# Parskatt/RoMa

Measured on AMD Instinct MI355X. Metric: image-pairs/sec, roma_outdoor 560->864, batch=8 per GPU, higher is better.
Workload: dtype bf16; 1 GPU; roma_outdoor match() 560->864, symmetric, upsample_preds, 8 pairs/GPU/step, seeded synthetic weights + N(0,1) images; precision policy of the reference's bf16 timing script: bfloat16 DINOv2 + float16 autocast for VGG / decoder / refiners (ROMA_MIXED), f32 accumulate; precision_policy=mixed, global_batch=8, streams_per_gpu=2, parallelism=single GPU, outputs_finite=True

## Files before the change

roma_amd/_lib.py:

```python
from __future__ import annotations

import ctypes as C
import os
import re

import torch

_PKG = os.path.dirname(os.path.abspath(__file__))
_HERE = os.environ.get("ROMA_LIB_DIR", _PKG)
LIB_PATH = os.path.join(_HERE, "libroma_hip.so")
LIB_PATHS = {"bf16": LIB_PATH, "f16": os.path.join(_HERE, "libroma_hip_f16.so")}

ROMA_F32, ROMA_BF16, ROMA_F16, ROMA_MIXED = 0, 1, 2, 3
H16_CODE = {"bf16": ROMA_BF16, "f16": ROMA_F16}


class RomaConfig(C.Structure):
    _fields_ = [("coarse_h", C.c_int), ("coarse_w", C.c_int), ("upsample_h", C.c_int), ("upsample_w", C.c_int),
                ("symmetric", C.c_int), ("upsample_preds", C.c_int), ("attenuate_cert", C.c_int),
                ("precision", C.c_int), ("max_batch", C.c_int), ("device", C.c_int)]


class RomaForwardArgs(C.Structure):
    _fields_ = [("upsample", C.c_int), ("symmetric", C.c_int), ("scale_factor", C.c_double),
                ("seed_flow", C.c_void_p), ("seed_cert", C.c_void_p), ("seed_h", C.c_int), ("seed_w", C.c_int),
                ("flow", C.c_void_p * 5), ("cert", C.c_void_p * 5), ("feat", C.c_void_p * 5)]


_CTYPES = {"int": C.c_int, "long": C.c_long, "float": C.c_float, "double": C.c_double, "long long": C.c_longlong,
           "unsigned long long": C.c_ulonglong, "roma_handle_t": C.c_void_p}


def _ctype(text, named, decl):
    words = re.findall(r"\w+|\*", text) if re.fullmatch(r"[\w\s*]+", text) else []
    if "*" in words:
        return C.c_char_p if [w for w in words[:words.index("*")] if w != "const"] == ["char"] else C.c_void_p
    key = " ".join(w for w in (words[:-1] if named else words) if w != "const")
    if key not in _CTYPES:
        raise ImportError(f"roma_hip.h: no ctypes type for `{' '.join(text.split())}` in `{decl}`")
    return _CTYPES[key]


def parse_header(text):
    text = re.sub(r"/\*.*?\*/|//[^\n]*", " ", text, flags=re.S)
    text = re.sub(r"^[ \t]*#.*$", " ", text, flags=re.M)
    text = re.sub(r"\b(typedef\s+struct|enum)\s*\{[^}]*\}[^;]*;|\btypedef\b[^;{]*;", " ", text)
    text = re.sub(r'extern\s+"C"\s*\{|\}', " ", text)
    sigs = {}
    for decl in filter(None, (" ".join(d.split()) for d in text.split(";"))):
        m = re.fullmatch(r"([\w\s*]+?)\s*\b(\w+)\s*\((.*)\)", decl)
        if not m:
            raise ImportError(f"roma_hip.h: `{decl}` is not a function declaration")
        ret, name, params = m.groups()
        sigs[name] = (_ctype(ret, False, decl), [_ctype(p, True, decl) for p in params.split(",") if params.strip() != "void"])
    return sigs


HEADER_PATH = os.path.join(os.path.dirname(_PKG), "include", "roma_hip.h")
if not os.path.exists(HEADER_PATH):
    raise ImportError(f"{HEADER_PATH} not found - roma_amd reads the signatures of the C ABI from it")
with open(HEADER_PATH) as _f:
    SIGNATURES = parse_header(_f.read())
EXTENSION_HEADERS = [os.path.join(os.path.dirname(_PKG), "include", "roma_hip_registration.h")]
EXTENSIONS = {}
for _path in EXTENSION_HEADERS:
    if not os.path.exists(_path):
        raise ImportError(f"{_path} not found - roma_amd reads the signatures of the C ABI from it")
    with open(_path) as _f:
        _sigs = parse_header(_f.read())
    _twice = sorted(set(_sigs) & (set(SIGNATURES) | set(EXTENSIONS)))
    if _twice:
        raise ImportError(f"{_path} declares {_twice} a second time")
    EXTENSIONS.update(_sigs)

_libs = {}


class RomaHipError(RuntimeError):
    pass


def load(fmt: str = "bf16"):
    if fmt in _libs:
        return _libs[fmt]
    path = LIB_PATHS[fmt]
    if not os.path.exists(path):
        raise ImportError(f"{path} not found - build it with `python -c 'import __graft_entry__ as g; g.build()'` "
                          "(roma_amd has no CPU fallback)")
    lib = C.CDLL(path)
    for name, (res, args) in {**SIGNATURES, **EXTENSIONS}.items():
        fn = getattr(lib, name)
        fn.restype = res
        fn.argtypes = args
    if lib.roma_h16_format() != H16_CODE[fmt]:
        raise ImportError(f"{path} does not store {fmt} (roma_h16_format() = {lib.roma_h16_format()})")
    lib.h16 = fmt
    _libs[fmt] = lib
    return lib


def fmt_of(dtype) -> str:
    return "f16" if str(dtype) == "torch.float16" else "bf16"


def last_error(lib=None) -> str:
    return (lib or load()).roma_last_error().decode("utf-8", "replace")


def check(rc: int, exc=RomaHipError, lib=None):
    if rc != 0:
        raise exc(last_error(lib))
    return rc


def _ptr(t):
    return C.c_void_p(t.data_ptr() if t is not None else 0)


def _stream(dev):
    return C.c_void_p(torch.cuda.current_stream(dev).cuda_stream)


def _device_tensor(x, name, module):
    if not isinstance(x, torch.Tensor) or not x.is_cuda:
        raise RomaHipError(f"roma_amd.{module}: {name} must be a tensor on a HIP device; there is no CPU fallback")
    return x.detach()
```

roma_amd/csrc/conv64.h:

```cpp
#pragma once
#include "gemm.h"

namespace roma {
int conv64_try_launch(const GemmArgs& a, hipStream_t stream);
int conv3x3_c3_bf16_launch(const float* img, const void* w, const float* bias, void* out, int B, int H, int W, hipStream_t stream);
}
```

roma_amd/csrc/conv64.hip:

```cpp
#include "conv64.h"

#include <stdio.h>
#include <stdlib.h>

#include <algorithm>

#include "gemm_device.h"
#include "tuning.h"

namespace roma {

static __device__ __attribute__((aligned(256))) unsigned int g_c64_dump[256];

#define C64_WAIT_VM(N) asm volatile("s_waitcnt vmcnt(%0)" ::"n"(N) : "memory")

template <int COUT>
__global__ __launch_bounds__(256, 2) void conv3x3_c64_kernel(const bf16_t* __restrict__ in, const bf16_t* __restrict__ w,
                                                             const float* __restrict__ bias, bf16_t* __restrict__ out, int B,
                                                             int H, int W, int SY, int nxt, int nblocks) {
  constexpr int NCG = COUT / 32;
  constexpr int NPG = 4 / NCG;
  constexpr int TW = 64 * NPG;
  constexpr int NPIECE = ((TW + 2) * 128 + 1023) / 1024;
  constexpr int RSTRIDE = NPIECE * 1024;
  constexpr int KW = (NPIECE + 3) / 4;
  extern __shared__ __attribute__((aligned(1024))) unsigned char ring[];

  if ((int)blockIdx.x >= nblocks) return;
  const int tid = threadIdx.x, lane = tid & 63;
  const int wave = __builtin_amdgcn_readfirstlane(tid >> 6);
  const int cg = wave % NCG, pg = wave / NCG;
  const int l31 = lane & 31, h = lane >> 5;
  typedef unsigned u32x4 __attribute__((ext_vector_type(4)));
  const unsigned ring0 = (unsigned)(size_t)((__attribute__((address_space(3))) unsigned char*)ring);

  u32x4 wreg[36];
  {
    const bf16_t* wp = w + (long)(32 * cg + l31) * 576 + 8 * h;
#pragma unroll
    for (int ks = 0; ks < 36; ++ks) wreg[ks] = *reinterpret_cast<const u32x4*>(wp + 16 * ks);
  }
  float* bias_s = reinterpret_cast<float*>(ring + 4 * RSTRIDE);
  if (tid < COUT) bias_s[tid] = bias[tid];

  unsigned rdo[3];
#pragma unroll
  for (int dx = 0; dx < 3; ++dx) {
    const int p = 64 * pg + l31 + dx;
    rdo[dx] = ring0 + (unsigned)(p * 128 + ((h ^ ((p >> 1) & 7)) << 4));
  }

  for (int lb = blockIdx.x; lb < nblocks; lb += gridDim.x) {
  const int xt = lb % nxt;
  const int r = lb / nxt;
  const int yt = (H + SY - 1) / SY;
  const int ys = (r % yt) * SY;
  const int b = r / yt;
  const int x0 = xt * TW;
  const int sy = min(SY, H - ys);
  if (lb != (int)blockIdx.x) __builtin_amdgcn_s_barrier();

  const bf16_t* inb = in + (long)b * H * W * 64;
  const __amdgpu_buffer_rsrc_t rs_in = __builtin_amdgcn_make_buffer_rsrc(const_cast<bf16_t*>(inb), 0, (int)((long)H * W * 128), 0x00020000);
  unsigned voff[KW];
  bool okx[KW];
  {
    const int dl_p = lane >> 3, dl_slot = lane & 7;
    const u32x4 z4 = {0u, 0u, 0u, 0u};
#pragma unroll
    for (int j = 0; j < KW; ++j) {
      const int q = wave + 4 * j;
      const int p = q * 8 + dl_p;
      const int x = x0 - 1 + p;
      const int c = dl_slot ^ ((p >> 1) & 7);
      okx[j] = q < NPIECE && p < TW + 2 && x >= 0 && x < W;
      voff[j] = okx[j] ? (unsigned)(x * 128 + c * 16) : 0u;
      if (q < NPIECE && !okx[j]) {
        int ln = lane;
        asm volatile("" : "+v"(ln));
#pragma unroll
        for (int sl = 0; sl < 4; ++sl)
          asm volatile("ds_write_b128 %0, %1" ::"v"(ring0 + sl * RSTRIDE + q * 1024 + ln * 16), "v"(z4) : "memory");
      }
    }
  }
  asm volatile("s_waitcnt vmcnt(0) lgkmcnt(0)" ::: "memory");

#define C64_ISSUE_ROW(YY, SLOT)                                                                                \
  {                                                                                                            \
    const int yy_ = (YY);                                                                                      \
    if (yy_ >= 0 && yy_ < H) {                                                                                 \
      const int so_ = yy_ * W * 128;                                                                           \
      _Pragma("unroll") for (int j = 0; j < KW; ++j) {                                                         \
        const int q_ = wave + 4 * j;                                                                           \
        if (q_ < NPIECE) {                                                                                     \
          if (okx[j])                                                                                          \
            __builtin_amdgcn_raw_ptr_buffer_load_lds(rs_in, (__attribute__((address_space(3))) void*)(ring + (SLOT) * RSTRIDE + q_ * 1024), \
                                                     16, (int)voff[j], so_, 0, 0);                             \
        }                                                                                                      \
      }                                                                                                        \
    } else {                                     \
      const u32x4 z4_ = {0u, 0u, 0u, 0u};                                                                      \
      int ln_ = lane;                                                                                          \
      asm volatile("" : "+v"(ln_));                                                                            \
      _Pragma("unroll") for (int j = 0; j < KW; ++j) {                                                         \
        const int q_ = wave + 4 * j;                                                                           \
        if (q_ < NPIECE)                                                                                       \
          asm volatile("ds_write_b128 %0, %1" ::"v"(ring0 + (SLOT) * RSTRIDE + q_ * 1024 + ln_ * 16), "v"(z4_) : "memory"); \
      }                                                                                                        \
    }                                                                                                          \
  }

  u32x4 fa[2][4];
#define C64_READ_G(SLOTOFF, DX, G)                                                                            \
  {                                                                                                           \
    const unsigned ad_ = (rdo[DX] + (SLOTOFF)) ^ (unsigned)((G) << 5);                                         \
    asm volatile("ds_read_b128 %0, %1" : "=v"(fa[0][G]) : "v"(ad_));                                           \
    asm volatile("ds_read_b128 %0, %1 offset:4096" : "=v"(fa[1][G]) : "v"(ad_));                              \
  }
#define C64_WAIT_G(G, N) asm volatile("s_waitcnt lgkmcnt(%2)" : "+v"(fa[0][G]), "+v"(fa[1][G]) : "n"(N) : "memory")

  C64_ISSUE_ROW(ys - 1, 0)
  C64_ISSUE_ROW(ys, 1)
  C64_ISSUE_ROW(ys + 1, 2)

  bf16_t* outb = out + (long)b * H * W * COUT;
  for (int o = 0; o < sy; ++o) {
    if (o == 0) {
      asm volatile("s_waitcnt vmcnt(0) lgkmcnt(0)" ::: "memory");
    } else {
      C64_WAIT_VM(0);
    }
    __builtin_amdgcn_s_barrier();
    C64_ISSUE_ROW(ys + o + 2, (o + 3) & 3)
    if (o == 0) {
      C64_READ_G(0, 0, 0)
      C64_READ_G(0, 0, 1)
    }
    C64_READ_G((o & 3) * RSTRIDE, 0, 2)
    C64_READ_G((o & 3) * RSTRIDE, 0, 3)

    f32x16 acc[2];
#pragma unroll
    for (int tm = 0; tm < 2; ++tm)
#pragma unroll
      for (int e = 0; e < 16; ++e) acc[tm][e] = 0.f;
#pragma unroll
    for (int t = 0; t < 9; ++t) {
#pragma unroll
      for (int g = 0; g < 4; ++g) {
        if (t == 8 && g == 3) {
          C64_WAIT_G(g, 4);
        } else {
          C64_WAIT_G(g, 6);
        }
#pragma unroll
        for (int tm = 0; tm < 2; ++tm)
          acc[tm] = mfma_h16_32x32x16(wreg[t * 4 + g],
                                                            fa[tm][g], acc[tm]);
        __builtin_amdgcn_sched_barrier(0);
        if (t + 1 < 9) {
          C64_READ_G(((o + (t + 1) / 3) & 3) * RSTRIDE, (t + 1) % 3, g)
        } else if (g < 2) {
          C64_READ_G(((o + 1) & 3) * RSTRIDE, 0, g)
        }
        __builtin_amdgcn_sched_barrier(0);
      }
    }

    const int y = ys + o;
#pragma unroll
    for (int P = 0; P < 2; ++P) {
      f32x4 bv0, bv1;
      {
        const unsigned ba = ring0 + 4 * RSTRIDE + (32 * cg + 16 * P + 4 * h) * 4;
        asm volatile("ds_read_b128 %0, %2\n\tds_read_b128 %1, %2 offset:32\n\ts_waitcnt lgkmcnt(0)"
                     : "=&v"(bv0), "=&v"(bv1)
                     : "v"(ba)
                     : "memory");
      }
#pragma unroll
      for (int tm = 0; tm < 2; ++tm) {
        const int x = x0 + 64 * pg + 32 * tm + l31;
        const unsigned a0 = pack_bf16x2(fmaxf(acc[tm][8 * P + 0] + bv0[0], 0.f), fmaxf(acc[tm][8 * P + 1] + bv0[1], 0.f));
        const unsigned a1 = pack_bf16x2(fmaxf(acc[tm][8 * P + 2] + bv0[2], 0.f), fmaxf(acc[tm][8 * P + 3] + bv0[3], 0.f));
        const unsigned b0 = pack_bf16x2(fmaxf(acc[tm][8 * P + 4] + bv1[0], 0.f), fmaxf(acc[tm][8 * P + 5] + bv1[1], 0.f));
        const unsigned b1 = pack_bf16x2(fmaxf(acc[tm][8 * P + 6] + bv1[2], 0.f), fmaxf(acc[tm][8 * P + 7] + bv1[3], 0.f));
        const auto s0 = __builtin_amdgcn_permlane32_swap(a0, b0, false, false);
        const auto s1 = __builtin_amdgcn_permlane32_swap(a1, b1, false, false);
        const u32x4 st = {s0[0], s1[0], s0[1], s1[1]};
        bf16_t* op = outb + ((long)y * W + x) * COUT + 32 * cg + 16 * P + 8 * h;
        u32x4* dst = x < W ? reinterpret_cast<u32x4*>(op) : reinterpret_cast<u32x4*>(g_c64_dump) + lane;
        *dst = st;
      }
    }
  }
  C64_WAIT_VM(0);
  }
#undef C64_WAIT_G
#undef C64_READ_G
#undef C64_ISSUE_ROW
}

template <int DUMMY>
__global__ __launch_bounds__(512, 1) void conv3x3_c128_kernel(const bf16_t* __restrict__ in, const bf16_t* __restrict__ w,
                                                              const float* __restrict__ bias, bf16_t* __restrict__ out, int B,
                                                              int H, int W, int SY, int nxt, int nblocks) {
  constexpr int COUT = 128, TW = 64;
  constexpr int NPIECE = ((TW + 2) * 256 + 1023) / 1024;
  constexpr int RSTRIDE = NPIECE * 1024;
  constexpr int KW = (NPIECE + 7) / 8;
  constexpr int XCH = 4 * RSTRIDE;
  constexpr int BIAS = XCH + 2 * 8 * 4096;
  extern __shared__ __attribute__((aligned(1024))) unsigned char ring[];
  if ((int)blockIdx.x >= nblocks) return;

  const int tid = threadIdx.x, lane = tid & 63;
  const int wave = __builtin_amdgcn_readfirstlane(tid >> 6);
  const int cg = wave & 3, kh = wave >> 2;
  const int l31 = lane & 31, h = lane >> 5;
  typedef unsigned u32x4 __attribute__((ext_vector_type(4)));
  const unsigned ring0 = (unsigned)(size_t)((__attribute__((address_space(3))) unsigned char*)ring);

  u32x4 wreg[36];
  {
    const bf16_t* wp = w + (long)(32 * cg + l31) * 1152 + 64 * kh + 8 * h;
#pragma unroll
    for (int t = 0; t < 9; ++t)
#pragma unroll
      for (int g = 0; g < 4; ++g) wreg[t * 4 + g] = *reinterpret_cast<const u32x4*>(wp + 128 * t + 16 * g);
  }
  float* bias_s = reinterpret_cast<float*>(ring + BIAS);
  if (tid < COUT) bias_s[tid] = bias[tid];

  unsigned rdo[3];
#pragma unroll
  for (int dx = 0; dx < 3; ++dx) {
    const int p = l31 + dx;
    rdo[dx] = ring0 + (unsigned)(p * 256 + (((8 * kh + h) ^ (p & 15)) << 4));
  }
  const unsigned xw = ring0 + XCH + (unsigned)((cg + 4 * (1 - kh)) * 4096 + lane * 16);
  const unsigned xr = ring0 + XCH + (unsigned)((cg + 4 * kh) * 4096 + lane * 16);

  for (int lb = blockIdx.x; lb < nblocks; lb += gridDim.x) {
  const int xt = lb % nxt;
  const int r = lb / nxt;
  const int yt = (H + SY - 1) / SY;
  const int ys = (r % yt) * SY;
  const int b = r / yt;
  const int x0 = xt * TW;
  const int sy = min(SY, H - ys);
  if (lb != (int)blockIdx.x) __builtin_amdgcn_s_barrier();

  const bf16_t* inb = in + (long)b * H * W * 128;
  const __amdgpu_buffer_rsrc_t rs_in = __builtin_amdgcn_make_buffer_rsrc(const_cast<bf16_t*>(inb), 0, (int)((long)H * W * 256), 0x00020000);
  unsigned voff[KW];
  bool okx[KW];
  {
    const int dl_p = lane >> 4, dl_slot = lane & 15;
    const u32x4 z4 = {0u, 0u, 0u, 0u};
#pragma unroll
    for (int j = 0; j < KW; ++j) {
      const int q = wave + 8 * j;
      const int p = q * 4 + dl_p;
      const int x = x0 - 1 + p;
      const int c = dl_slot ^ (p & 15);
      okx[j] = q < NPIECE && p < TW + 2 && x >= 0 && x < W;
      voff[j] = okx[j] ? (unsigned)(x * 256 + c * 16) : 0u;
      if (q < NPIECE && !okx[j]) {
        int ln = lane;
        asm volatile("" : "+v"(ln));
#pragma unroll
        for (int sl = 0; sl < 4; ++sl)
          asm volatile("ds_write_b128 %0, %1" ::"v"(ring0 + sl * RSTRIDE + q * 1024 + ln * 16), "v"(z4) : "memory");
      }
    }
  }
  asm volatile("s_waitcnt vmcnt(0) lgkmcnt(0)" ::: "memory");

#define C128_ISSUE_ROW(YY, SLOT)                                                                               \
  {                                                                                                            \
    const int yy_ = (YY);                                                                                      \
    if (yy_ >= 0 && yy_ < H) {                                                                                 \
      const int so_ = yy_ * W * 256;                                                                           \
      _Pragma("unroll") for (int j = 0; j < KW; ++j) {                                                         \
        const int q_ = wave + 8 * j;                                                                           \
        if (q_ < NPIECE) {                                                                                     \
          if (okx[j])                                                                                          \
            __builtin_amdgcn_raw_ptr_buffer_load_lds(rs_in, (__attribute__((address_space(3))) void*)(ring + (SLOT) * RSTRIDE + q_ * 1024), \
                                                     16, (int)voff[j], so_, 0, 0);                             \
        }                                                                                                      \
      }                                                                                                        \
    } else {                                                                                                   \
      const u32x4 z4_ = {0u, 0u, 0u, 0u};                                                                      \
      int ln_ = lane;                                                                                          \
      asm volatile("" : "+v"(ln_));                                                                            \
      _Pragma("unroll") for (int j = 0; j < KW; ++j) {                                                         \
        const int q_ = wave + 8 * j;                                                                           \
        if (q_ < NPIECE)                                                                                       \
          asm volatile("ds_write_b128 %0, %1" ::"v"(ring0 + (SLOT) * RSTRIDE + q_ * 1024 + ln_ * 16), "v"(z4_) : "memory"); \
      }                                                                                                        \
    }                                                                                                          \
  }

  u32x4 fa[2][4];
#define C128_READ_G(SLOTOFF, DX, G)                                                                           \
  {                                                                                                           \
    const unsigned ad_ = (rdo[DX] + (SLOTOFF)) ^ (unsigned)((G) << 5);                                         \
    asm volatile("ds_read_b128 %0, %1" : "=v"(fa[0][G]) : "v"(ad_));                                           \
    asm volatile("ds_read_b128 %0, %1 offset:8192" : "=v"(fa[1][G]) : "v"(ad_));                              \
  }
#define C128_WAIT_G(G, N) asm volatile("s_waitcnt lgkmcnt(%2)" : "+v"(fa[0][G]), "+v"(fa[1][G]) : "n"(N) : "memory")

  bf16_t* outb = out + (long)b * H * W * COUT;
#define C128_EPILOGUE(ACC, Y, PAR)                                                                            \
  {                                                                                                           \
    f32x4 pp_[4];                                                                                             \
    asm volatile("ds_read_b128 %0, %4\n\tds_read_b128 %1, %4 offset:1024\n\tds_read_b128 %2, %4 offset:2048\n\t" \
                 "ds_read_b128 %3, %4 offset:3072\n\ts_waitcnt lgkmcnt(0)"                                    \
                 : "=&v"(pp_[0]), "=&v"(pp_[1]), "=&v"(pp_[2]), "=&v"(pp_[3])                                 \
                 : "v"(xr + (unsigned)(PAR) * 32768u)                                                         \
                 : "memory");                                                                                 \
    const int x_ = x0 + 32 * kh + l31;                                                                        \
    _Pragma("unroll") for (int P = 0; P < 2; ++P) {                                                           \
      f32x4 bv0_, bv1_;                                                                                       \
      asm volatile("ds_read_b128 %0, %2\n\tds_read_b128 %1, %2 offset:32\n\ts_waitcnt lgkmcnt(0)"            \
                   : "=&v"(bv0_), "=&v"(bv1_)                                                                 \
                   : "v"(ring0 + BIAS + (32 * cg + 16 * P + 4 * h) * 4)                                       \
                   : "memory");                                                                               \
      const f32x4 p0_ = pp_[2 * P], p1_ = pp_[2 * P + 1];                                                     \
      const unsigned a0_ = pack_bf16x2(fmaxf(ACC[8 * P + 0] + p0_[0] + bv0_[0], 0.f), fmaxf(ACC[8 * P + 1] + p0_[1] + bv0_[1], 0.f)); \
      const unsigned a1_ = pack_bf16x2(fmaxf(ACC[8 * P + 2] + p0_[2] + bv0_[2], 0.f), fmaxf(ACC[8 * P + 3] + p0_[3] + bv0_[3], 0.f)); \
      const unsigned b0_ = pack_bf16x2(fmaxf(ACC[8 * P + 4] + p1_[0] + bv1_[0], 0.f), fmaxf(ACC[8 * P + 5] + p1_[1] + bv1_[1], 0.f)); \
      const unsigned b1_ = pack_bf16x2(fmaxf(ACC[8 * P + 6] + p1_[2] + bv1_[2], 0.f), fmaxf(ACC[8 * P + 7] + p1_[3] + bv1_[3], 0.f)); \
      const auto s0_ = __builtin_amdgcn_permlane32_swap(a0_, b0_, false, false);                              \
      const auto s1_ = __builtin_amdgcn_permlane32_swap(a1_, b1_, false, false);                              \
      const u32x4 st_ = {s0_[0], s1_[0], s0_[1], s1_[1]};                                                     \
      bf16_t* op_ = outb + ((long)(Y) * W + x_) * COUT + 32 * cg + 16 * P + 8 * h;                            \
      u32x4* dst_ = x_ < W ? reinterpret_cast<u32x4*>(op_) : reinterpret_cast<u32x4*>(g_c64_dump) + lane;     \
      *dst_ = st_;                                                                                            \
    }                                                                                                         \
  }
#define C128_PUBLISH(ACC, PAR)                                                                                \
  _Pragma("unroll") for (int j = 0; j < 4; ++j) {                                                             \
    const f32x4 v_ = {ACC[4 * j + 0], ACC[4 * j + 1], ACC[4 * j + 2], ACC[4 * j + 3]};                        \
    asm volatile("ds_write_b128 %0, %1" ::"v"(xw + (unsigned)(PAR) * 32768u + j * 1024), "v"(v_) : "memory"); \
  }

  C128_ISSUE_ROW(ys - 1, 0)
  C128_ISSUE_ROW(ys, 1)
  C128_ISSUE_ROW(ys + 1, 2)

  f32x16 acc[2];
  for (int o = 0; o < sy; ++o) {
    asm volatile("s_waitcnt vmcnt(0) lgkmcnt(0)" ::: "memory");
    __builtin_amdgcn_s_barrier();
    if (o > 0) {
      if (kh == 0) C128_EPILOGUE(acc[0], ys + o - 1, (o - 1) & 1)
      else C128_EPILOGUE(acc[1], ys + o - 1, (o - 1) & 1)
    }
    C128_ISSUE_ROW(ys + o + 2, (o + 3) & 3)
    if (o == 0) {
      C128_READ_G(0, 0, 0)
      C128_READ_G(0, 0, 1)
    }
    C128_READ_G((o & 3) * RSTRIDE, 0, 2)
    C128_READ_G((o & 3) * RSTRIDE, 0, 3)

#pragma unroll
    for (int tm = 0; tm < 2; ++tm)
#pragma unroll
      for (int e = 0; e < 16; ++e) acc[tm][e] = 0.f;
#pragma unroll
    for (int t = 0; t < 9; ++t) {
#pragma unroll
      for (int g = 0; g < 4; ++g) {
        if (t == 8 && g == 3) {
          C128_WAIT_G(g, 4);
        } else {
          C128_WAIT_G(g, 6);
        }
#pragma unroll
        for (int tm = 0; tm < 2; ++tm)
          acc[tm] = mfma_h16_32x32x16(wreg[t * 4 + g],
                                                            fa[tm][g], acc[tm]);
        __builtin_amdgcn_sched_barrier(0);
        if (t + 1 < 9) {
          C128_READ_G(((o + (t + 1) / 3) & 3) * RSTRIDE, (t + 1) % 3, g)
        } else if (g < 2) {
          C128_READ_G(((o + 1) & 3) * RSTRIDE, 0, g)
        }
        __builtin_amdgcn_sched_barrier(0);
      }
    }
    if (kh == 0) C128_PUBLISH(acc[1], o & 1)
    else C128_PUBLISH(acc[0], o & 1)
  }
  asm volatile("s_waitcnt vmcnt(0) lgkmcnt(0)" ::: "memory");
  __builtin_amdgcn_s_barrier();
  if (kh == 0) C128_EPILOGUE(acc[0], ys + sy - 1, (sy - 1) & 1)
  else C128_EPILOGUE(acc[1], ys + sy - 1, (sy - 1) & 1)
  C64_WAIT_VM(0);
  }
#undef C128_PUBLISH
#undef C128_EPILOGUE
#undef C128_WAIT_G
#undef C128_READ_G
#undef C128_ISSUE_ROW
}

__global__ __launch_bounds__(256, 4) void conv3x3_c3_bf16_kernel(const float* __restrict__ img, const bf16_t* __restrict__ w,
                                                                 const float* __restrict__ bias, bf16_t* __restrict__ out, int B,
                                                                 int H, int W, int RY, int nxt, long ntiles) {
  __shared__ __attribute__((aligned(16))) float bias_s[64];
  __shared__ __attribute__((aligned(1024))) unsigned char stage[4][4096];
  if (threadIdx.x < 64) bias_s[threadIdx.x] = bias[threadIdx.x];
  __syncthreads();
  const int lane = threadIdx.x & 63;
  const int wave = __builtin_amdgcn_readfirstlane(threadIdx.x >> 6);
  const long t = (long)blockIdx.x * 4 + wave;
  if (t >= ntiles) return;
  const int xt = (int)(t % nxt);
  const long r = t / nxt;
  const int nyb = (H + RY - 1) / RY;
  const int y0 = (int)(r % nyb) * RY;
  const int b = (int)(r / nyb);
  const int l31 = lane & 31, h = lane >> 5;
  const int x = xt * 32 + l31;
  const int HW = H * W;
  typedef unsigned u32x4 __attribute__((ext_vector_type(4)));

  u32x4 wf[2][2];
#pragma unroll
  for (int cb = 0; cb < 2; ++cb)
#pragma unroll
    for (int ks = 0; ks < 2; ++ks) wf[cb][ks] = *reinterpret_cast<const u32x4*>(w + (32 * cb + l31) * 32 + 16 * h + 8 * ks);

  int toff[16], tsel[16];
#pragma unroll
  for (int s_ = 0; s_ < 16; ++s_) {
    const int k0 = s_, k1 = 16 + s_;
    const int o0 = (k0 / 9) * HW + ((k0 % 9) / 3 - 1) * W + (k0 % 3 - 1);
    const int o1 = k1 < 27 ? (k1 / 9) * HW + ((k1 % 9) / 3 - 1) * W + (k1 % 3 - 1) : 0;
    const int m0 = (1 << ((k0 % 9) / 3)) | (8 << (k0 % 3));
    const int m1 = k1 < 27 ? ((1 << ((k1 % 9) / 3)) | (8 << (k1 % 3))) : 64;
    toff[s_] = h ? o1 : o0;
    tsel[s_] = h ? m1 : m0;
  }
  const int colbits = ((x >= 1 && x - 1 < W) ? 8 : 0) | (x < W ? 16 : 0) | (x + 1 < W ? 32 : 0);
  const bool cols_in = xt * 32 >= 1 && xt * 32 + 33 <= W;
  const float* p0 = img + (long)b * 3 * HW;
  bf16_t* outb = out + (long)b * HW * 64;
  const unsigned st0 = (unsigned)(size_t)((__attribute__((address_space(3))) unsigned char*)stage[wave]);
  const int ny = min(RY, H - y0);
  for (int o = 0; o < ny; ++o) {
    const int y = y0 + o;
    const int base = y * W + x;
    float v[16];
    if (cols_in && y >= 1 && y + 1 < H) {
#pragma unroll
      for (int s_ = 0; s_ < 16; ++s_) v[s_] = p0[base + toff[s_]];
      if (h) {
#pragma unroll
        for (int s_ = 11; s_ < 16; ++s_) v[s_] = 0.f;
      }
    } else {
      const int okbits = colbits | (y >= 1 ? 1 : 0) | 2 | (y + 1 < H ? 4 : 0);
#pragma unroll
      for (int s_ = 0; s_ < 16; ++s_) {
        const bool ok = (okbits & tsel[s_]) == tsel[s_];
        const float ld = p0[ok ? base + toff[s_] : 0];
        v[s_] = ok ? ld : 0.f;
      }
    }
    u32x4 fr[2];
#pragma unroll
    for (int ks = 0; ks < 2; ++ks)
#pragma unroll
      for (int j = 0; j < 4; ++j) fr[ks][j] = pack_bf16x2(v[8 * ks + 2 * j], v[8 * ks + 2 * j + 1]);
    f32x16 acc[2];
#pragma unroll
    for (int cb = 0; cb < 2; ++cb) {
#pragma unroll
      for (int e = 0; e < 16; ++e) acc[cb][e] = 0.f;
#pragma unroll
      for (int ks = 0; ks < 2; ++ks)
        acc[cb] = mfma_h16_32x32x16(wf[cb][ks],
                                                          fr[ks], acc[cb]);
    }
#pragma unroll
    for (int cb = 0; cb < 2; ++cb)
#pragma unroll
      for (int P = 0; P < 2; ++P) {
        const f32x4 b0 = *reinterpret_cast<const f32x4*>(bias_s + 32 * cb + 16 * P + 4 * h);
        const f32x4 b1 = *reinterpret_cast<const f32x4*>(bias_s + 32 * cb + 16 * P + 8 + 4 * h);
        const unsigned a0 = pack_bf16x2(fmaxf(acc[cb][8 * P + 0] + b0[0], 0.f), fmaxf(acc[cb][8 * P + 1] + b0[1], 0.f));
        const unsigned a1 = pack_bf16x2(fmaxf(acc[cb][8 * P + 2] + b0[2], 0.f), fmaxf(acc[cb][8 * P + 3] + b0[3], 0.f));
        const unsigned c0 = pack_bf16x2(fmaxf(acc[cb][8 * P + 4] + b1[0], 0.f), fmaxf(acc[cb][8 * P + 5] + b1[1], 0.f));
        const unsigned c1 = pack_bf16x2(fmaxf(acc[cb][8 * P + 6] + b1[2], 0.f), fmaxf(acc[cb][8 * P + 7] + b1[3], 0.f));
        const auto s0 = __builtin_amdgcn_permlane32_swap(a0, c0, false, false);
        const auto s1 = __builtin_amdgcn_permlane32_swap(a1, c1, false, false);
        const u32x4 st = {s0[0], s1[0], s0[1], s1[1]};
        const int c = 4 * cb + 2 * P + h;
        *reinterpret_cast<__attribute__((address_space(3))) u32x4*>(st0 + l31 * 128 + ((c ^ (l31 & 7)) << 4)) = st;
      }
#pragma unroll
    for (int i = 0; i < 4; ++i) {
      const u32x4 st = *reinterpret_cast<__attribute__((address_space(3))) const u32x4*>(st0 + i * 1024 + lane * 16);
      const int px = i * 8 + (lane >> 3);
      const int c = (lane & 7) ^ (px & 7);
      if (xt * 32 + px < W) *reinterpret_cast<u32x4*>(outb + ((long)y * W + xt * 32 + px) * 64 + c * 8) = st;
    }
  }
}

int conv3x3_c3_bf16_launch(const float* img, const void* w, const float* bias, void* out, int B, int H, int W, hipStream_t stream) {
  ROMA_REQUIRE(img && w && bias && out && B > 0 && H > 0 && W > 0, "conv3x3_c3_bf16: bad arguments");
  ROMA_REQUIRE((long)3 * H * W < (1l << 23), "conv3x3_c3_bf16: image too large for the packed tap offsets");
  const int RY = 8;
  const int nxt = (W + 31) / 32;
  const long ntiles = (long)B * ((H + RY - 1) / RY) * nxt;
  ProfScope ps("conv3x3_c3_bf16_kernel", (double)B * H * W * (12.0 + 128.0), "byte", stream);
  hipLaunchKernelGGL(conv3x3_c3_bf16_kernel, dim3((unsigned)((ntiles + 3) / 4)), dim3(256), 0, stream, img,
                     reinterpret_cast<const bf16_t*>(w), bias, reinterpret_cast<bf16_t*>(out), B, H, W, RY, nxt, ntiles);
  ROMA_LAUNCH_CHECK();
  return 0;
}

int conv64_try_launch(const GemmArgs& a, hipStream_t stream) {
  const int use = tuning(SW_CONV64);
  const bool c128 = a.conv_c == 128;
  if (!(use & (c128 ? 2 : 1))) return 1;
  if ((a.conv_c != 64 && !c128) || a.in_dt != DT_BF16 || a.out_dt != DT_BF16 || a.act != ACT_RELU || !a.bias) return 1;
  if (c128 ? a.N != 128 : (a.N != 64 && a.N != 128)) return 1;
  if (a.ldc != a.N || a.ldw != 9 * a.conv_c || a.batch != 1 || a.mode != EPI_STD || a.scale || a.res || a.res_bf16 || a.alpha != 1.0f)
    return 1;
  const int H = a.conv_h, W = a.conv_w;
  const long hw = (long)H * W;
  if (hw <= 0 || a.M % hw != 0) return 1;
  if ((long)hw * a.conv_c * 2 >= (1l << 31)) return 1;
  const int B = (int)(a.M / hw);
  const int TW = (!c128 && a.N == 64) ? 128 : 64;
  const int slots = c128 ? 256 : 512;
  const int sy_env = tuning(SW_CONV64_SY);
  const int nxt = (W + TW - 1) / TW;
  int SY = sy_env;
  if (SY <= 0) {
    long best = -1;
    for (int yt = 1; yt <= std::max(1, H / 12); ++yt) {
      const int sy = (H + yt - 1) / yt;
      const long n = (long)B * nxt * ((H + sy - 1) / sy);
      const long cost = ((n + slots - 1) / slots) * (sy + 3);
      if (best < 0 || cost < best) {
        best = cost;
        SY = sy;
      }
    }
  }
  const long nb = (long)B * ((H + SY - 1) / SY) * nxt;
  if (nb <= 0 || nb >= (1l << 30)) return 1;
  char pname[64];
  snprintf(pname, sizeof pname, c128 ? "conv3x3_c128_kernel<%d>" : "conv3x3_c64_kernel<%d>", a.N);
  ProfScope ps(pname, 2.0 * (double)a.M * a.N * 9.0 * a.conv_c, "flop", stream);
  const bf16_t* in = reinterpret_cast<const bf16_t*>(a.A);
  const bf16_t* w = reinterpret_cast<const bf16_t*>(a.W);
  bf16_t* out = reinterpret_cast<bf16_t*>(a.C);
  constexpr int LDS64 = 4 * 17 * 1024 + 512, LDS64N128 = 4 * 9 * 1024 + 512;
  constexpr int LDS128 = 4 * 17 * 1024 + 2 * 8 * 4096 + 512;
  static bool attr_set[64] = {false};
  int dev = 0;
  ROMA_CHECK_HIP(hipGetDevice(&dev));
  if (dev < 0 || dev >= 64 || !attr_set[dev]) {
    ROMA_CHECK_HIP(hipFuncSetAttribute(reinterpret_cast<const void*>(&conv3x3_c64_kernel<64>), hipFuncAttributeMaxDynamicSharedMemorySize, LDS64));
    ROMA_CHECK_HIP(hipFuncSetAttribute(reinterpret_cast<const void*>(&conv3x3_c64_kernel<128>), hipFuncAttributeMaxDynamicSharedMemorySize, LDS64N128));
    ROMA_CHECK_HIP(hipFuncSetAttribute(reinterpret_cast<const void*>(&conv3x3_c128_kernel<0>), hipFuncAttributeMaxDynamicSharedMemorySize, LDS128));
    if (dev >= 0 && dev < 64) attr_set[dev] = true;
  }
  const long gx = std::min<long>(nb, slots);
  if (c128) {
    hipLaunchKernelGGL(conv3x3_c128_kernel<0>, dim3((unsigned)gx), dim3(512), LDS128, stream, in, w, a.bias, out, B, H, W, SY, nxt, (int)nb);
  } else if (a.N == 64) {
    hipLaunchKernelGGL(conv3x3_c64_kernel<64>, dim3((unsigned)gx), dim3(256), LDS64, stream, in, w, a.bias, out, B, H, W, SY, nxt, (int)nb);
  } else {
    hipLaunchKernelGGL(conv3x3_c64_kernel<128>, dim3((unsigned)gx), dim3(256), LDS64N128, stream, in, w, a.bias, out, B, H, W, SY, nxt, (int)nb);
  }
  ROMA_LAUNCH_CHECK();
  return 0;
}

}
```

roma_amd/csrc/model.hip:

```cpp
#include "model.h"

#include <dlfcn.h>
#include <math.h>
#include <stdlib.h>

#include <algorithm>

#include "arch.h"
#include "attention.h"
#include "conv64.h"
#include "dry_run.h"
#include "pool_proj.h"
#include "elementwise.h"
#include "gemm.h"
#include "gp.h"
#include "local_corr.h"
#include "refiner_block.h"
#include "vit.h"

namespace roma {

std::mutex g_peer_mutex;
extern void* g_peer_lib;
extern int g_mixed_handles;

Model::~Model() {
  for (int i = 0; i < MAX_STREAMS - 1; ++i) {
    if (side[i]) (void)hipStreamDestroy(side[i]);
    if (ev_join[i]) (void)hipEventDestroy(ev_join[i]);
  }
  if (ev_fork) (void)hipEventDestroy(ev_fork);
  for (void* p : owned) (void)hipFree(p);
  for (auto& kv : dbg) (void)hipFree(kv.second.first);
  for (auto& kv : inject) (void)hipFree(kv.second.first);
  if (peer_lib) {
    std::lock_guard<std::mutex> lk(g_peer_mutex);
    --g_mixed_handles;
  }
}


int Model::load_peer() {
  static void* lib = nullptr;
  static int (*fwd)(const roma_vit_args_t*, void*) = nullptr;
  std::lock_guard<std::mutex> lk(g_peer_mutex);
  if (!lib) {
    ROMA_REQUIRE(roma_h16_format() == ROMA_F16, "ROMA_MIXED is a mode of the binary16 build (libroma_hip_f16.so)");
    Dl_info info;
    ROMA_REQUIRE(dladdr(reinterpret_cast<void*>(&roma_vit_forward), &info) && info.dli_fname, "ROMA_MIXED: cannot locate this library");
    std::string path(info.dli_fname);
    const size_t slash = path.find_last_of('/');
    path = (slash == std::string::npos ? std::string("") : path.substr(0, slash + 1)) + "libroma_hip.so";
    void* l = dlopen(path.c_str(), RTLD_NOW | RTLD_LOCAL | RTLD_DEEPBIND);
    if (!l) {
      set_error("ROMA_MIXED: cannot load the bfloat16 library " + path + ": " + (dlerror() ? dlerror() : "?"));
      return ROMA_ERR_STATE;
    }
    auto fmt = reinterpret_cast<int (*)(void)>(dlsym(l, "roma_h16_format"));
    auto self = reinterpret_cast<int (*)(void)>(dlsym(l, "roma_self_check"));
    auto abi = reinterpret_cast<int (*)(void)>(dlsym(l, "roma_abi_stamp"));
    auto f = reinterpret_cast<int (*)(const roma_vit_args_t*, void*)>(dlsym(l, "roma_vit_forward"));
    std::string why;
    if (!fmt || !f || !self || !abi) why = "it does not export roma_h16_format / roma_self_check / roma_abi_stamp / roma_vit_forward (an older build)";
    else if (fmt() != ROMA_BF16) why = "it is not the bfloat16 build";
    else if (abi() != roma_abi_stamp()) why = "its ABI stamp " + std::to_string(abi()) + " differs from this library's " + std::to_string(roma_abi_stamp()) + " (stale build: roma_vit_args_t would be misread)";
    else if (self() != ROMA_BF16) why = "its internal calls resolve into another library (symbol interposition: link both builds with -Wl,-Bsymbolic)";
    if (!why.empty()) {
      dlclose(l);
      set_error("ROMA_MIXED: " + path + " cannot serve as the bfloat16 sibling: " + why);
      return ROMA_ERR_STATE;
    }
    lib = l;
    fwd = f;
    g_peer_lib = l;
  }
  if (!peer_lib) ++g_mixed_handles;
  peer_lib = lib;
  peer_vit_forward = fwd;
  return 0;
}

int Model::debug_inject(const char* name, const void* host, size_t bytes) {
  ROMA_REQUIRE(name, "roma_debug_inject: null name");
  const std::string k(name);
  ROMA_REQUIRE(k == "gm_flow16" || k == "gm_cert16", "roma_debug_inject: unknown stage (gm_flow16, gm_cert16)");
  ROMA_CHECK_HIP(hipSetDevice(cfg.device));
  auto it = inject.find(k);
  if (it != inject.end()) {
    ROMA_CHECK_HIP(hipDeviceSynchronize());
    (void)hipFree(it->second.first);
    inject.erase(it);
  }
  if (!host || bytes == 0) return 0;
  void* p = nullptr;
  ROMA_CHECK_HIP(hipMalloc(&p, bytes));
  ROMA_CHECK_HIP(hipMemcpy(p, host, bytes, hipMemcpyHostToDevice));
  inject[k] = {p, bytes};
  return 0;
}

int Model::finalize() {
  ROMA_REQUIRE(!finalized, "roma_finalize: already finalized");
  ROMA_CHECK_HIP(hipSetDevice(cfg.device));
  if (int rc = check_contract()) return rc;
  act_dt = cfg.precision == ROMA_F32 ? DT_F32 : DT_BF16;
  mixed = cfg.precision == ROMA_MIXED;
  if (mixed)
    if (int rc = load_peer()) return rc;
  if (int rc = pack_weights()) return rc;
  host.clear();
  arena.dry = persist.dry = true;
  arena.peak = persist.peak = 0;
  const int keep_sym = cfg.symmetric, keep_up = cfg.upsample_preds;
  cfg.symmetric = 1;
  cfg.upsample_preds = cfg.upsample_h > 0 ? 1 : 0;
  int rc = match_impl(cfg.max_batch, nullptr, nullptr, nullptr, nullptr, nullptr, nullptr, nullptr, true, arena, persist);
  int cf[5];
  for (int i = 0; i < 5; ++i) cf[i] = ref[i].Cf;
  pack = pack_layout(cfg.coarse_h, cfg.coarse_w, cfg.upsample_h, cfg.upsample_w, cf, act_dt == DT_F32 ? 4 : 2);
  const EncodedIn plan_enc;
  if (!rc) rc = match_impl(cfg.max_batch, nullptr, nullptr, nullptr, nullptr, nullptr, nullptr, nullptr, true, arena, persist, nullptr, &plan_enc);
  if (!rc) rc = encode_impl(2 * cfg.max_batch, nullptr, nullptr, nullptr, nullptr, true, cfg.upsample_h > 0, arena, persist);
  Arena plan, plan_p;
  if (!rc && cfg.max_batch >= 2)
    rc = match_impl(cfg.max_batch / 2, nullptr, nullptr, nullptr, nullptr, nullptr, nullptr, nullptr, true, plan, plan_p);
  if (!rc && cfg.max_batch >= 2)
    rc = match_impl(cfg.max_batch / 2, nullptr, nullptr, nullptr, nullptr, nullptr, nullptr, nullptr, true, plan, plan_p, nullptr, &plan_enc);
  cfg.symmetric = keep_sym;
  cfg.upsample_preds = keep_up;
  if (rc) return rc;
  side_arena_bytes = plan.peak + 4096;
  side_persist_bytes = plan_p.peak + 4096;
  arena.cap = arena.peak + 4096;
  persist.cap = persist.peak + 4096;
  ROMA_CHECK_HIP(hipMalloc((void**)&arena.base, arena.cap));
  owned.push_back(arena.base);
  ROMA_CHECK_HIP(hipMalloc((void**)&persist.base, persist.cap));
  owned.push_back(persist.base);
  ROMA_CHECK_HIP(hipMemset(persist.base, 0, persist.cap));
  ROMA_CHECK_HIP(hipMemset(arena.base, 0, arena.cap));
  arena.dry = persist.dry = false;
  finalized = true;
  return 0;
}

int Model::ensure_side_streams(int n) {
  for (int i = streams_ready - 1; i + 1 < n; ++i) {
    Arena &a = side_arena[i], &p = side_persist[i];
    a.cap = side_arena_bytes;
    p.cap = side_persist_bytes;
    ROMA_CHECK_HIP(hipMalloc((void**)&a.base, a.cap));
    owned.push_back(a.base);
    ROMA_CHECK_HIP(hipMalloc((void**)&p.base, p.cap));
    owned.push_back(p.base);
    ROMA_CHECK_HIP(hipMemset(p.base, 0, p.cap));
    ROMA_CHECK_HIP(hipMemset(a.base, 0, a.cap));
    ROMA_CHECK_HIP(hipDeviceSynchronize());
    a.dry = p.dry = false;
    ROMA_CHECK_HIP(hipStreamCreateWithFlags(&side[i], hipStreamNonBlocking));
    ROMA_CHECK_HIP(hipEventCreateWithFlags(&ev_join[i], hipEventDisableTiming));
    if (!ev_fork) ROMA_CHECK_HIP(hipEventCreateWithFlags(&ev_fork, hipEventDisableTiming));
    streams_ready = i + 2;
  }
  return 0;
}

static int dbg_dual_slot() { return tuning(SW_DEBUG_DUAL_SLOT); }

int Model::dbg_save(const char* name, const void* p, size_t bytes, hipStream_t st) {
  if (!debug) return 0;
  if (dbg_dual_slot() >= 0) {
    static const std::string only = std::string(",") + (getenv("ROMA_DEBUG_ONLY") ? getenv("ROMA_DEBUG_ONLY") : "") + ",";
    if (dbg_cur_slot != dbg_dual_slot() || only.find(std::string(",") + name + ",") == std::string::npos) return 0;
  }
  auto it = dbg.find(name);
  if (it == dbg.end() || it->second.second != bytes) {
    if (it != dbg.end()) (void)hipFree(it->second.first);
    void* q = nullptr;
    ROMA_CHECK_HIP(hipMalloc(&q, bytes));
    dbg[name] = {q, bytes};
    it = dbg.find(name);
  }
  ROMA_CHECK_HIP(hipMemcpyAsync(it->second.first, p, bytes, hipMemcpyDeviceToDevice, st));
  return 0;
}

int Model::match(int B, const float* ima, const float* imb, const float* ima_hr, const float* imb_hr, float* warp,
                 float* cert, hipStream_t st) {
  ROMA_REQUIRE(finalized, "roma_match: call roma_finalize first");
  ROMA_REQUIRE(B >= 1 && B <= cfg.max_batch, "roma_match: batch size out of range (max_batch)");
  ROMA_REQUIRE(ima && imb && warp && cert, "roma_match: null image / output pointer");
  if (cfg.upsample_preds) {
    ROMA_REQUIRE(cfg.upsample_h > 0, "roma_match: upsample_preds set but the handle has no upsample resolution");
    ROMA_REQUIRE(ima_hr && imb_hr, "roma_match: upsample_preds requires im_A_high_res and im_B_high_res");
  }
  ROMA_CHECK_HIP(hipSetDevice(cfg.device));
  return match_streams(B, ima, imb, ima_hr, imb_hr, warp, cert, st);
}

int Model::forward(int B, const float* ima, const float* imb, const roma_forward_args_t* fw, hipStream_t st) {
  ROMA_REQUIRE(finalized, "roma_forward: call roma_finalize first");
  ROMA_REQUIRE(B >= 1 && B <= cfg.max_batch, "roma_forward: batch size out of range (max_batch)");
  ROMA_REQUIRE(ima && imb && fw, "roma_forward: null image / argument pointer");
  if (fw->upsample) {
    ROMA_REQUIRE(cfg.upsample_h > 0, "roma_forward: upsample pass on a handle without an upsample resolution");
    ROMA_REQUIRE(fw->seed_flow && fw->seed_cert && fw->seed_h > 0 && fw->seed_w > 0,
                 "roma_forward: the upsample pass needs batch[\"corresps\"] (seed_flow / seed_cert)");
  }
  ROMA_CHECK_HIP(hipSetDevice(cfg.device));
  return match_impl(B, ima, imb, nullptr, nullptr, nullptr, nullptr, st, false, arena, persist, fw);
}

int Model::encode(int N, const float* images, const float* images_hr, void* feats, long feats_bytes, hipStream_t st) {
  ROMA_REQUIRE(finalized, "roma_encode: call roma_finalize first");
  ROMA_REQUIRE(N >= 1 && images && feats, "roma_encode: N < 1 or null image / feature pointer");
  ROMA_REQUIRE(!images_hr || cfg.upsample_h > 0, "roma_encode: high-resolution images on a handle without an upsample resolution");
  ROMA_REQUIRE(feats_bytes == (long)N * pack.total, "roma_encode: feats_bytes must be N * roma_encoded_bytes() = " +
                                                        std::to_string((long)N * pack.total) + " (got " + std::to_string(feats_bytes) + ")");
  ROMA_REQUIRE((reinterpret_cast<uintptr_t>(feats) & 15) == 0, "roma_encode: the feature buffer must be 16-byte aligned");
  ROMA_CHECK_HIP(hipSetDevice(cfg.device));
  const size_t im_lo = (size_t)3 * cfg.coarse_h * cfg.coarse_w, im_hi = (size_t)3 * cfg.upsample_h * cfg.upsample_w;
  const int chunk = 2 * cfg.max_batch;
  for (int i0 = 0; i0 < N; i0 += chunk)
    if (int rc = encode_impl(std::min(chunk, N - i0), images + i0 * im_lo, images_hr ? images_hr + i0 * im_hi : nullptr,
                             static_cast<char*>(feats) + (long)i0 * pack.total, st, false, images_hr != nullptr, arena, persist))
      return rc;
  return 0;
}

int Model::match_encoded(int P, const void* feats, long feats_bytes, int N, const int* idx_a, const int* idx_b, float* warp, float* cert,
                         hipStream_t st) {
  ROMA_REQUIRE(finalized, "roma_match_encoded: call roma_finalize first");
  ROMA_REQUIRE(P >= 1 && P <= cfg.max_batch, "roma_match_encoded: number of pairs out of range (max_batch)");
  ROMA_REQUIRE(feats && idx_a && idx_b && warp && cert && N >= 1, "roma_match_encoded: null pointer or N < 1");
  ROMA_REQUIRE(feats_bytes == (long)N * pack.total, "roma_match_encoded: feats_bytes must be N * roma_encoded_bytes() = " +
                                                        std::to_string((long)N * pack.total) + " (got " + std::to_string(feats_bytes) + ")");
  ROMA_REQUIRE((reinterpret_cast<uintptr_t>(feats) & 15) == 0, "roma_match_encoded: the feature buffer must be 16-byte aligned");
  for (int i = 0; i < P; ++i)
    ROMA_REQUIRE(idx_a[i] >= 0 && idx_a[i] < N && idx_b[i] >= 0 && idx_b[i] < N,
                 "roma_match_encoded: pair " + std::to_string(i) + " = (" + std::to_string(idx_a[i]) + ", " + std::to_string(idx_b[i]) +
                     ") names an image outside [0, " + std::to_string(N) + ")");
  if (cfg.upsample_preds)
    ROMA_REQUIRE(cfg.upsample_h > 0, "roma_match_encoded: upsample_preds set but the handle has no upsample resolution");
  ROMA_CHECK_HIP(hipSetDevice(cfg.device));
  const EncodedIn enc{static_cast<const char*>(feats), idx_a, idx_b};
  return match_streams(P, nullptr, nullptr, nullptr, nullptr, warp, cert, st, &enc);
}

int Model::match_streams(int B, const float* ima, const float* imb, const float* ima_hr, const float* imb_hr, float* warp,
                         float* cert, hipStream_t st, const EncodedIn* enc) {
  const int env_streams = tuning(SW_STREAMS);
  const bool serial_env = tuning(SW_STREAMS_SERIAL) != 0;
  const int ns = (debug && dbg_dual_slot() < 0) ? 1 : std::min(std::min(env_streams > 0 ? env_streams : n_streams, (int)MAX_STREAMS), B);
  if (ns <= 1) return match_impl(B, ima, imb, ima_hr, imb_hr, warp, cert, st, false, arena, persist, nullptr, enc);
  if (int rc = ensure_side_streams(ns)) return rc;
  const size_t im_lo = (size_t)3 * cfg.coarse_h * cfg.coarse_w, im_hi = (size_t)3 * cfg.upsample_h * cfg.upsample_w;
  const int Ho = cfg.upsample_preds ? cfg.upsample_h : cfg.coarse_h, Wo = cfg.upsample_preds ? cfg.upsample_w : cfg.coarse_w;
  const size_t px = (size_t)Ho * Wo * (cfg.symmetric ? 2 : 1);
  ROMA_CHECK_HIP(hipEventRecord(ev_fork, st));
  int rc = 0, b0 = 0;
  for (int i = 0; i < ns; ++i) {
    const int bi = B / ns + (i < B % ns ? 1 : 0);
    hipStream_t si = i == 0 ? st : side[i - 1];
    if (i > 0) ROMA_CHECK_HIP(hipStreamWaitEvent(si, ev_fork, 0));
    if (i > 0 && serial_env) {
      hipStream_t sp = i == 1 ? st : side[i - 2];
      ROMA_CHECK_HIP(hipEventRecord(ev_join[i - 1], sp));
      ROMA_CHECK_HIP(hipStreamWaitEvent(si, ev_join[i - 1], 0));
    }
    EncodedIn sub;
    if (enc) sub = EncodedIn{enc->feats, enc->idx_a + b0, enc->idx_b + b0};
    if (!rc)
      rc = match_impl(bi, ima ? ima + b0 * im_lo : nullptr, imb ? imb + b0 * im_lo : nullptr, ima_hr ? ima_hr + b0 * im_hi : nullptr,
                      imb_hr ? imb_hr + b0 * im_hi : nullptr, warp + b0 * px * 4, cert + b0 * px, si, false,
                      i == 0 ? arena : side_arena[i - 1], i == 0 ? persist : side_persist[i - 1], nullptr, enc ? &sub : nullptr);
    b0 += bi;
  }
  for (int i = 1; i < ns; ++i) {
    (void)hipEventRecord(ev_join[i - 1], side[i - 1]);
    (void)hipStreamWaitEvent(st, ev_join[i - 1], 0);
  }
  return rc;
}

struct Model::Call {
  Arena &arena, &persist;
  int B = 0, nimg = 0, ndp = 0;
  int shift = 0;
  bool sym = false;
  size_t esz = 4;
  hipStream_t st = nullptr;
  bool dry = false;
  int tslot = 0;
  bool tracing = false;
  const roma_forward_args_t* fw = nullptr;
  int th = 0, tw = 0, T = 0;
  int Npd = 0, Npt = 0;
  void *qbuf = nullptr, *kbuf = nullptr, *vtbuf = nullptr;
  void *ln = nullptr, *ao = nullptr, *hid = nullptr;
  Call(Arena& a, Arena& p) : arena(a), persist(p) {}
  void* alloc(size_t elems, size_t es) const { return arena.alloc(elems * es); }
  void* at(void* p, long elems) const { return static_cast<char*>(p) + elems * (long)esz; }
};

struct Model::Pass {
  bool up = false;
  int H = 0, W = 0;
  const float *imA = nullptr, *imB = nullptr;
  void* feat[5] = {nullptr};
  void* pf_pre[2] = {nullptr, nullptr};
  bool pp_on[2] = {false, false};
  double scale_factor = 1.0;
  float *flow = nullptr, *cert = nullptr, *flow_alt = nullptr, *cert_alt = nullptr;
  const char* tag() const { return up ? "p2" : "p1"; }
};

struct Model::Scale {
  int si, ins, hs, ws;
  int lvl;
  long hw, M;
  const RefinerW& r;
  int ldf;
  float sx, sy;
  std::string tp;
  size_t pf_bytes, d_bytes, flow_bytes, cert_bytes;
  void* pf = nullptr;
  void *d0 = nullptr, *d1 = nullptr;
  Scale(const Call& c, const Pass& p, int si_, const RefinerW& r_)
      : si(si_), ins(SCALE_INT[si_]), hs(ins == 16 ? c.th : p.H / ins), ws(ins == 16 ? c.tw : p.W / ins),
        lvl(ins == 16 ? 4 : (ins == 8 ? 3 : (ins == 4 ? 2 : (ins == 2 ? 1 : 0)))), hw((long)hs * ws), M((long)c.ndp * hw), r(r_),
        ldf((int)round_up(r_.Cf, 8)), sx((float)ins / (4.0f * (float)p.W)), sy((float)ins / (4.0f * (float)p.H)),
        tp(std::string(p.tag()) + "_s" + SCALES[si_]), pf_bytes((size_t)c.nimg * hw * ldf * c.esz),
        d_bytes((size_t)M * r_.Cp * c.esz), flow_bytes((size_t)M * 2 * 4), cert_bytes((size_t)M * 4) {}
};

int Model::fits(const Call& c) {
  if (c.dry || !(c.arena.overflow || c.persist.overflow)) return 0;
  c.arena.overflow = c.persist.overflow = false;
  set_error("roma_match / roma_forward: the workspace planned by roma_finalize is too small for this call (an option that "
            "changes the buffer plan was switched after roma_finalize); the results of this call are invalid");
  return -5;
}

int Model::observe(const Call& c, const std::string& trace_name, const std::string& dbg_name, const void* p, size_t bytes,
                   long rows, int ld, int c0, int c1) {
  if (c.tracing && !trace_name.empty() && trace_n[c.tslot] < TRACE_MAX) {
    const int k = trace_n[c.tslot]++;
    if ((int)trace_names[c.tslot].size() <= k) trace_names[c.tslot].push_back(trace_name);
    else trace_names[c.tslot][k] = trace_name;
    unsigned long long* out = trace_dev[c.tslot] + k;
    if (int rc = c1 > c0 ? checksum_cols_launch(p, rows, ld, c0, c1, out, c.st) : checksum_launch(p, bytes, out, c.st)) return rc;
  }
  if (debug && !c.dry && !dbg_name.empty()) return dbg_save(dbg_name.c_str(), p, bytes, c.st);
  return 0;
}

int Model::encode_vgg(const Call& c, Pass& p) {
  const bool dry = c.dry; hipStream_t st = c.st;
  const int H = p.H, W = p.W, nimg = c.nimg, B = c.B;
  const size_t esz = c.esz;
  const int fh[4] = {H, H / 2, H / 4, H / 8}, fw_[4] = {W, W / 2, W / 4, W / 8};
  const int fc[4] = {64, 128, 256, 512};
  size_t fbytes[4];
  for (int l = 0; l < 4; ++l) {
    fbytes[l] = (size_t)nimg * fh[l] * fw_[l] * fc[l] * esz;
    p.feat[l] = c.arena.alloc(fbytes[l]);
  }
  const int pp_si[2] = {4, 3};
  for (int l = 0; l < 2; ++l) {
    const RefinerW& rr = ref[pp_si[l]];
    const int ldf_l = (int)round_up(rr.Cf, 8);
    p.pp_on[l] = tuning(SW_POOL_PROJ) != 0 && fh[l] >= 2 && fw_[l] >= 2 &&
                 pool_proj_supported(fc[l], rr.Cf, ldf_l, act_dt) && proj[pp_si[l]].b != nullptr;
    if (p.pp_on[l] || dry) p.pf_pre[l] = c.alloc((size_t)nimg * fh[l] * fw_[l] * ldf_l, esz);
    if (!p.pp_on[l] && !dry) p.pf_pre[l] = nullptr;
  }
  const size_t enc_mark = c.arena.mark();
  void* t0 = c.alloc((size_t)nimg * H * W * 64, esz);
  void* t1 = c.alloc((size_t)nimg * (H / 2) * (W / 2) * 64, esz);
  void* col1 = c.alloc((size_t)nimg * H * W * 32, esz);
  if (int rc = fits(c)) return rc;
  if (act_dt == DT_BF16 && (tuning(SW_CONV64) & 4) && (long)3 * H * W < (1l << 23)) {
    RUN(conv3x3_c3_bf16_launch(p.imA, vgg[0].w, vgg[0].b, t0, B, H, W, st));
    if (p.imB) RUN(conv3x3_c3_bf16_launch(p.imB, vgg[0].w, vgg[0].b, c.at(t0, (long)B * H * W * 64), B, H, W, st));
  } else {
    RUN(im2col3x3_c3_launch(p.imA, col1, B, H, W, act_dt, st));
    if (p.imB) RUN(im2col3x3_c3_launch(p.imB, c.at(col1, (long)B * H * W * 32), B, H, W, act_dt, st));
    GemmArgs g;
    g.A = col1; g.lda = 32; g.W = vgg[0].w; g.ldw = vgg[0].ldw; g.C = t0; g.ldc = 64;
    g.M = nimg * H * W; g.N = 64; g.K = 32; g.k_alg = 27; g.in_dt = act_dt; g.out_dt = act_dt; g.bias = vgg[0].b; g.act = ACT_RELU;
    RUN(gemm_launch(g, st));
  }
  auto conv = [&](int li, const void* in, void* out, int h, int w) -> int {
    GemmArgs g;
    g.A = in; g.W = vgg[li].w; g.ldw = vgg[li].ldw; g.C = out; g.ldc = vgg_cout[li];
    g.M = nimg * h * w; g.N = vgg_cout[li]; g.K = 9 * vgg_cin[li];
    g.in_dt = act_dt; g.out_dt = act_dt; g.bias = vgg[li].b; g.act = ACT_RELU;
    g.conv_h = h; g.conv_w = w; g.conv_c = vgg_cin[li]; g.conv_korder = vgg_korder[li];
    RUN(gemm_launch(g, st));
    return 0;
  };
  auto pool = [&](int l, const void* in, void* out) -> int {
    if (p.pp_on[l]) {
      const int si_ = pp_si[l];
      RUN(pool_proj_launch(in, out, p.pf_pre[l], proj[si_].w, proj[si_].ldw, proj[si_].b, ref[si_].Cf, (int)round_up(ref[si_].Cf, 8),
                           nimg, fh[l], fw_[l], fc[l], act_dt, st));
    } else {
      RUN(maxpool2x2_launch(in, out, nimg, fh[l], fw_[l], fc[l], act_dt, st));
    }
    return 0;
  };
  if (int rc = conv(1, t0, p.feat[0], H, W)) return rc;
  if (int rc = pool(0, p.feat[0], t1)) return rc;
  if (int rc = conv(2, t1, t0, H / 2, W / 2)) return rc;
  if (int rc = conv(3, t0, p.feat[1], H / 2, W / 2)) return rc;
  if (int rc = pool(1, p.feat[1], t1)) return rc;
  if (int rc = conv(4, t1, t0, H / 4, W / 4)) return rc;
  if (int rc = conv(5, t0, t1, H / 4, W / 4)) return rc;
  if (int rc = conv(6, t1, t0, H / 4, W / 4)) return rc;
  if (int rc = conv(7, t0, p.feat[2], H / 4, W / 4)) return rc;
  RUN(maxpool2x2_launch(p.feat[2], t1, nimg, H / 4, W / 4, 256, act_dt, st));
  if (int rc = conv(8, t1, t0, H / 8, W / 8)) return rc;
  if (int rc = conv(9, t0, t1, H / 8, W / 8)) return rc;
  if (int rc = conv(10, t1, t0, H / 8, W / 8)) return rc;
  if (int rc = conv(11, t0, p.feat[3], H / 8, W / 8)) return rc;
  c.arena.release(enc_mark);
  static const char* const dbg_names[4] = {"feat1", "feat2", "feat4", "feat8"};
  for (int l = 0; l < 4; ++l)
    if (int rc = observe(c, std::string(p.tag()) + "_" + dbg_names[l], p.up ? "" : dbg_names[l], p.feat[l], fbytes[l])) return rc;
  if (c.fw && !dry)
    for (int l = 0; l < 4; ++l)
      if (c.fw->feat[4 - l]) ROMA_CHECK_HIP(hipMemcpyAsync(c.fw->feat[4 - l], p.feat[l], fbytes[l], hipMemcpyDeviceToDevice, st));
  return 0;
}

int Model::encode_dino(Call& c, Pass& p) {
  const bool dry = c.dry; hipStream_t st = c.st;
  const int nimg = c.nimg, T = c.T;
  const size_t esz = c.esz;
  const long rows_d = (long)nimg * (T + 1), rows_t = (long)c.ndp * T;
  const size_t fbytes = (size_t)nimg * T * 1024 * esz;
  p.feat[4] = c.arena.alloc(fbytes);
  const long rmax = std::max(rows_d, rows_t);
  c.ln = c.alloc((size_t)rmax * 1024, esz);
  c.ao = c.alloc((size_t)rmax * 1024, esz);
  c.hid = c.alloc((size_t)rmax * 4096, esz);
  const size_t dmark = c.arena.mark();
  void* col = c.alloc((size_t)nimg * T * patch.ldw, esz);
  float* pt = (float*)c.alloc((size_t)nimg * T * 1024, 4);
  float* x = (float*)c.alloc((size_t)rows_d * 1024, 4);
  const bool res_f32_env = tuning(SW_VIT_RES_F32) != 0;
  void* xs = nullptr;
  if (act_dt == DT_BF16) xs = c.alloc((size_t)rows_d * 1024, 2);
  void* feat_vit = p.feat[4];
  if (mixed) feat_vit = c.alloc((size_t)nimg * T * 1024, 2);
  if (int rc = fits(c)) return rc;
  if (!dry) {
    roma_vit_block_t blk[24];
    for (int i = 0; i < 24; ++i) blk[i] = dino[i].pub();
    roma_vit_args_t va{};
    va.B = c.B; va.H = p.H; va.W = p.W;
    va.act = act_dt == DT_F32 ? ROMA_F32 : (mixed ? ROMA_BF16 : roma_h16_format());
    va.bf16_residual = act_dt == DT_BF16 && vit_bf16_residual && !res_f32_env;
    va.im_a = p.imA; va.im_b = p.imB;
    va.patch_w = patch.w; va.patch_b = patch.b; va.patch_ldw = patch.ldw;
    va.cls_tok = cls_tok; va.pos_emb = pos_emb;
    va.blocks = blk; va.nblocks = 24;
    va.norm_w = dino_nw; va.norm_b = dino_nb;
    va.col = col; va.pt = pt; va.x = x; va.xs = xs; va.ln = c.ln; va.ao = c.ao; va.hid = c.hid;
    va.q = c.qbuf; va.k = c.kbuf; va.vt = c.vtbuf;
    va.feat_out = feat_vit;
    if (mixed) {
      if (int rc = peer_vit_forward(&va, st)) {
        set_error("ROMA_MIXED: roma_vit_forward of the bfloat16 library failed");
        return rc;
      }
      RUN(convert_from_bf16_launch(feat_vit, p.feat[4], (long)nimg * T * 1024, st));
    } else {
      RUN(vit_forward(va, st));
    }
  }
  c.arena.release(dmark);
  if (int rc = observe(c, "feat16", "feat16", p.feat[4], fbytes)) return rc;
  if (c.fw && !dry && c.fw->feat[0]) ROMA_CHECK_HIP(hipMemcpyAsync(c.fw->feat[0], p.feat[4], fbytes, hipMemcpyDeviceToDevice, st));
  return 0;
}

int Model::seed_upsample_pass(const Call& c, const Pass& p, const float* flow_p1, const float* cert_p1) {
  const bool dry = c.dry;
  const roma_forward_args_t* fw = c.fw;
  const int sh = fw ? fw->seed_h : cfg.coarse_h, sw = fw ? fw->seed_w : cfg.coarse_w;
  RUN(resize_bilinear_launch(fw ? fw->seed_flow : flow_p1, p.flow, c.ndp, sh, sw, p.H / 8, p.W / 8, 2, c.st));
  RUN(resize_bilinear_launch(fw ? fw->seed_cert : cert_p1, p.cert, c.ndp, sh, sw, p.H / 8, p.W / 8, 1, c.st));
  return 0;
}

int Model::proj_head(const Call& c, const Pass& p, Scale& s) {
  const bool dry = c.dry;
  const bool pf_ready = s.lvl < 2 && p.pp_on[s.lvl];
  s.pf = pf_ready ? p.pf_pre[s.lvl] : c.arena.alloc(s.pf_bytes);
  if (int rc = fits(c)) return rc;
  if (!pf_ready) {
    GemmArgs g;
    g.A = p.feat[s.lvl]; g.lda = PROJ_CIN[s.si]; g.W = proj[s.si].w; g.ldw = proj[s.si].ldw; g.C = s.pf; g.ldc = s.ldf;
    g.M = (int)(c.nimg * s.hw); g.N = s.r.Cf; g.K = PROJ_CIN[s.si]; g.in_dt = act_dt; g.out_dt = act_dt; g.bias = proj[s.si].b;
    RUN(gemm_launch(g, c.st));
  }
  return observe(c, s.tp + "_proj", s.ins == 16 ? "proj16" : "", s.pf, s.pf_bytes);
}

int Model::coarse_match(const Call& c, const Pass& p, const Scale& s) {
  const bool dry = c.dry; hipStream_t st = c.st;
  const long rows_t = s.M;
  float* tokens = (float*)c.alloc((size_t)rows_t * 1024, 4);
  const size_t gp_mark = c.arena.mark();
  if (int rc = gp_posterior(s.pf, s.ldf, act_dt, c.B, c.sym, c.th, c.tw, gp_w, gp_b, tokens, 1024, c.arena, st, dry))
    return c.arena.overflow ? fits(c) : rc;
  c.arena.release(gp_mark);
  const int ldl = 4104;
  float* logits = (float*)c.alloc((size_t)rows_t * ldl, 4);
  if (int rc = fits(c)) return rc;
  RUN(copy2d_launch(s.pf, s.ldf, act_dt, tokens + 512, 1024, DT_F32, rows_t, 512, st));
  if (int rc = observe(c, "", "tokens16", tokens, (size_t)rows_t * 1024 * 4)) return rc;
  VitScratch sc;
  sc.ln = c.ln; sc.ao = c.ao; sc.hid = c.hid; sc.q = c.qbuf; sc.k = c.kbuf; sc.vt = c.vtbuf;
  for (int i = 0; i < 5; ++i) RUN(vit_block_run(tdec[i].pub(), tokens, DT_F32, rows_t, c.ndp, c.T, c.Npt, 8, 128, 1e-5f, act_dt, sc, st));
  const void* zin = tokens;
  if (act_dt != DT_F32) {
    RUN(copy2d_launch(tokens, 1024, DT_F32, c.ln, 1024, act_dt, rows_t, 1024, st));
    zin = c.ln;
  }
  GemmArgs g;
  g.A = zin; g.lda = 1024; g.W = to_out.w; g.ldw = to_out.ldw; g.C = logits; g.ldc = ldl;
  g.M = (int)rows_t; g.N = to_out.N; g.K = 1024; g.in_dt = act_dt; g.out_dt = DT_F32; g.bias = to_out.b;
  RUN(gemm_launch(g, st));
  if (int rc = observe(c, s.tp + "_tokens_gp", "", tokens, (size_t)rows_t * 1024 * 4)) return rc;
  if (int rc = observe(c, s.tp + "_logits", "logits16", logits, (size_t)rows_t * ldl * 4)) return rc;
  RUN(cls_to_flow_launch(logits, ldl, p.flow, p.cert, rows_t, st));
  if (int rc = observe(c, s.tp + "_gm_flow", "gm_flow16_own", p.flow, s.flow_bytes)) return rc;
  if (!debug || dry) return 0;
  auto inj = [&](const char* nm, float* dst, size_t bytes) -> int {
    auto it = inject.find(nm);
    if (it == inject.end()) return 0;
    ROMA_REQUIRE(it->second.second == bytes, "roma_debug_inject: injected stage has the wrong size for this batch");
    ROMA_CHECK_HIP(hipMemcpyAsync(dst, it->second.first, bytes, hipMemcpyDeviceToDevice, st));
    return 0;
  };
  if (int rc = inj("gm_flow16", p.flow, s.flow_bytes)) return rc;
  if (int rc = inj("gm_cert16", p.cert, s.cert_bytes)) return rc;
  if (int rc = observe(c, "", "gm_flow16", p.flow, s.flow_bytes)) return rc;
  return observe(c, "", "gm_cert16", p.cert, s.cert_bytes);
}

int Model::refiner_input(const Call& c, const Pass& p, Scale& s) {
  const bool dry = c.dry; hipStream_t st = c.st;
  const RefinerW& r = s.r;
  s.d0 = c.arena.alloc(s.d_bytes);
  s.d1 = c.arena.alloc(s.d_bytes);
  LocalCorrArgs lc;
  if (r.radius) {
    const long lc_ints = local_corr_ws_ints(c.ndp, s.hs, s.ws, r.radius);
    lc.ws = (int*)c.alloc((size_t)lc_ints, 4); lc.ws_bytes = lc_ints * 4;
  }
  if (int rc = fits(c)) return rc;
  if (int rc = observe(c, s.tp + "_flow_before", "", p.flow, s.flow_bytes)) return rc;
  RefinerInputArgs ia;
  ia.feat = s.pf; ia.ldf = s.ldf; ia.flow = p.flow; ia.d = s.d0; ia.ldd = r.Cp; ia.emb_w = r.emb_w; ia.emb_b = r.emb_b;
  ia.B = c.ndp; ia.H = s.hs; ia.W = s.ws; ia.C = r.Cf; ia.E = r.E; ia.Kcorr = r.K; ia.nimg = c.nimg; ia.shift = c.shift;
  ia.disp_scale = (float)(40.0 / 32.0 * p.scale_factor); ia.dt = act_dt;
  RUN(refiner_input_launch(ia, st));
  if (r.radius) {
    lc.f0 = s.pf; lc.f1 = s.pf; lc.warp = p.flow; lc.out = c.at(s.d0, 2 * r.Cf + r.E);
    lc.B = c.ndp; lc.H = s.hs; lc.W = s.ws; lc.C = r.Cf; lc.radius = r.radius; lc.ld0 = s.ldf; lc.ld1 = s.ldf; lc.ldo = r.Cp;
    lc.nimg = c.nimg; lc.f1_shift = c.shift; lc.scale = 1.0f / sqrtf((float)r.Cf); lc.in_dt = act_dt; lc.out_dt = act_dt;
    RUN(local_corr_window_launch(lc, st));
  }
  const bool dual = dbg_dual_slot() >= 0;
  const bool din_small = s.d_bytes <= ((size_t)(dual ? 512 : 64) << 20);
  if (int rc = observe(c, s.tp + "_din", din_small ? std::string(p.tag()) + "_din" + SCALES[s.si] : "", s.d0, s.d_bytes)) return rc;
  if (dual && s.ins == 1)
    if (int rc = observe(c, "", std::string(p.tag()) + "_flowin1", p.flow, s.flow_bytes)) return rc;
  if (!c.tracing) return 0;
  if (int rc = observe(c, s.tp + "_proj_again", "", s.pf, s.pf_bytes)) return rc;
  if (int rc = observe(c, s.tp + "_flow_again", "", p.flow, s.flow_bytes)) return rc;
  if (int rc = observe(c, s.tp + "_din_again", "", s.d0, s.d_bytes)) return rc;
  if (c.esz != 2 || r.E <= 0) return 0;
  const int cols[5] = {0, r.Cf, 2 * r.Cf, 2 * r.Cf + r.E, r.Cp};
  static const char* const part[4] = {"_din_x", "_din_xhat", "_din_emb", "_din_rest"};
  for (int i = 0; i < 4; ++i)
    if (int rc = observe(c, s.tp + part[i], "", s.d0, 0, s.M, r.Cp, cols[i], cols[i + 1])) return rc;
  for (int b = 0; b < c.ndp; ++b)
    if (int rc = observe(c, s.tp + "_din_pair" + std::to_string(b), "", c.at(s.d0, (long)b * s.hw * r.Cp), 0, s.hw, r.Cp, 0, r.Cp)) return rc;
  return 0;
}

int Model::refiner_chain(const Call& c, const Pass& p, const Scale& s, const void** d_last, bool* composed) {
  const bool dry = c.dry; hipStream_t st = c.st;
  const RefinerW& r = s.r;
  const bool fused = fuse_refiner_blocks && refiner_block_supported(r.Cp, act_dt);
  float* delta = fused && (dry || compose_out_conv) ? (float*)c.alloc((size_t)s.M * 4, 4) : nullptr;
  if (int rc = fits(c)) return rc;
  void *dcur = s.d0, *dalt = s.d1;
  *composed = compose_out_conv;
  for (int b = 0; b < 9; ++b) {
    const bool last = b == 8 && compose_out_conv;
    if (last && fused) {
      RUN(refiner_block_final_launch(dcur, delta, r.dw_w[b], r.dw_b[b], r.ocf_w, r.Cp, r.ocf_b, c.ndp, s.hs, s.ws, r.Cp, act_dt, st));
      RUN(refiner_apply_delta_launch(delta, p.flow, p.cert, s.M, s.sx, s.sy, st));
      *d_last = nullptr;
      return 0;
    }
    if (fused) {
      RUN(refiner_block_launch(dcur, dalt, r.dw_w[b], r.dw_b[b], r.pw[b].w, r.pw[b].ldw, r.pw[b].b, c.ndp, s.hs, s.ws, r.Cp, act_dt, st));
      std::swap(dcur, dalt);
      if (int rc = observe(c, s.tp + "_blk" + std::to_string(b), "", dcur, s.d_bytes)) return rc;
      continue;
    }
    RUN(dwconv5x5_launch(dcur, dalt, r.dw_w[b], r.dw_b[b], c.ndp, s.hs, s.ws, r.Cp, act_dt, st));
    if (int rc = observe(c, s.tp + "_dw" + std::to_string(b), "", dalt, s.d_bytes)) return rc;
    if (last) {
      std::swap(dcur, dalt);
      break;
    }
    GemmArgs g;
    g.A = dalt; g.lda = r.Cp; g.W = r.pw[b].w; g.ldw = r.pw[b].ldw; g.C = dcur; g.ldc = r.Cp;
    g.M = (int)s.M; g.N = r.Cp; g.K = r.Cp; g.in_dt = act_dt; g.out_dt = act_dt; g.bias = r.pw[b].b;
    g.n_alg = g.k_alg = r.C;
    RUN(gemm_launch(g, st));
    if (int rc = observe(c, s.tp + "_blk" + std::to_string(b), "", dcur, s.d_bytes)) return rc;
  }
  *d_last = dcur;
  return 0;
}

int Model::refiner_out(const Call& c, const Pass& p, const Scale& s, const void* d_last, bool composed) {
  const bool dry = c.dry; hipStream_t st = c.st;
  const RefinerW& r = s.r;
  if (d_last)
    RUN(refiner_out_launch(d_last, r.Cp, act_dt, composed ? r.oc_w : r.out_w, composed ? r.oc_b : r.out_b, p.flow, p.cert, s.M, r.Cp,
                           s.sx, s.sy, st));
  if (int rc = observe(c, s.tp + "_flow", std::string(p.tag()) + "_flow" + SCALES[s.si], p.flow, s.flow_bytes)) return rc;
  if (int rc = observe(c, s.tp + "_cert", std::string(p.tag()) + "_cert" + SCALES[s.si], p.cert, s.cert_bytes)) return rc;
  if (c.fw && !dry) {
    if (c.fw->flow[s.si]) ROMA_CHECK_HIP(hipMemcpyAsync(c.fw->flow[s.si], p.flow, s.flow_bytes, hipMemcpyDeviceToDevice, st));
    if (c.fw->cert[s.si]) ROMA_CHECK_HIP(hipMemcpyAsync(c.fw->cert[s.si], p.cert, s.cert_bytes, hipMemcpyDeviceToDevice, st));
  }
  return 0;
}

int Model::next_scale(const Call& c, Pass& p, const Scale& s, float* cert16_keep) {
  const bool dry = c.dry; hipStream_t st = c.st;
  if (s.ins == 16) {
    if (s.M % 4 == 0) {
      RUN(copy2d_launch(p.cert, s.M, DT_F32, cert16_keep, s.M, DT_F32, 1, (int)s.M, st));
    } else if (!dry) {
      ROMA_CHECK_HIP(hipMemcpyAsync(cert16_keep, p.cert, s.cert_bytes, hipMemcpyDeviceToDevice, st));
    }
  }
  if (s.ins == 1) return 0;
  const int nh = p.H / (s.ins / 2), nw = p.W / (s.ins / 2);
  RUN(resize_bilinear_launch(p.flow, p.flow_alt, c.ndp, s.hs, s.ws, nh, nw, 2, st));
  RUN(resize_bilinear_launch(p.cert, p.cert_alt, c.ndp, s.hs, s.ws, nh, nw, 1, st));
  std::swap(p.flow, p.flow_alt);
  std::swap(p.cert, p.cert_alt);
  return observe(c, s.tp + "_flow_up", "", p.flow, (size_t)c.ndp * nh * nw * 2 * 4);
}

int Model::epilogue(const Call& c, const float* flow, const float* cert, const float* cert16_keep, float* warp_out, float* cert_out) {
  const bool dry = c.dry;
  const int Hfin = cfg.upsample_preds ? cfg.upsample_h : cfg.coarse_h, Wfin = cfg.upsample_preds ? cfg.upsample_w : cfg.coarse_w;
  FinalArgs fa;
  fa.flow = flow;
  fa.cert = cert;
  fa.cert16 = cfg.attenuate_cert ? cert16_keep : nullptr;
  fa.warp = warp_out; fa.certainty = cert_out;
  fa.B = c.B; fa.H = Hfin; fa.W = Wfin; fa.h16 = c.th; fa.w16 = c.tw; fa.symmetric = cfg.symmetric;
  RUN(final_epilogue_launch(fa, c.st));
  const size_t px = (size_t)c.B * Hfin * Wfin * (cfg.symmetric ? 2 : 1);
  if (int rc = observe(c, "final_warp", "", warp_out, px * 4 * 4)) return rc;
  return observe(c, "final_cert", "", cert_out, px * 4);
}

void Model::token_grid(Call& c) {
  c.th = cfg.coarse_h / 14; c.tw = cfg.coarse_w / 14; c.T = c.th * c.tw;
  c.Npd = (int)round_up(c.T + 1, 128); c.Npt = (int)round_up(c.T, 128);
  const size_t qkv_elems = std::max((size_t)c.nimg * 16 * c.Npd * 64, (size_t)c.ndp * 8 * c.Npt * 128);
  c.qbuf = c.persist.alloc(qkv_elems * c.esz);
  c.kbuf = c.persist.alloc(qkv_elems * c.esz);
  c.vtbuf = c.persist.alloc(qkv_elems * c.esz);
}

int Model::decoder_scratch(Call& c) {
  const long rows_t = (long)c.ndp * c.T;
  c.ln = c.alloc((size_t)rows_t * 1024, c.esz);
  c.ao = c.alloc((size_t)rows_t * 1024, c.esz);
  c.hid = c.alloc((size_t)rows_t * 4096, c.esz);
  return fits(c);
}

int Model::gather_head(const Call& c, const Pass& p, Scale& s, const EncodedIn& enc) {
  const bool dry = c.dry;
  s.pf = c.arena.alloc(s.pf_bytes);
  if (int rc = fits(c)) return rc;
  const long seg = pack.off[p.up ? 1 : 0][s.si], slab = pack.bytes[p.up ? 1 : 0][s.si];
  ROMA_REQUIRE(seg >= 0 && (size_t)slab * c.nimg == s.pf_bytes, "roma_match_encoded: the pack layout does not hold this scale");
  for (int i0 = 0; i0 < c.nimg && !dry; i0 += SLAB_MAX) {
    SlabTable t;
    t.n = std::min((int)SLAB_MAX, c.nimg - i0);
    for (int k = 0; k < t.n; ++k) {
      const int i = i0 + k;
      t.src_idx[k] = i < c.B ? enc.idx_a[i] : enc.idx_b[i - c.B];
      t.dst_idx[k] = i;
    }
    RUN(slab_copy_launch(enc.feats + seg, pack.total, s.pf, slab, slab, t, c.st));
  }
  return observe(c, s.tp + "_proj", s.ins == 16 ? "proj16" : "", s.pf, s.pf_bytes);
}

int Model::scatter_head(const Call& c, const Pass& p, const Scale& s, char* feats) {
  const bool dry = c.dry;
  const long seg = pack.off[p.up ? 1 : 0][s.si], slab = pack.bytes[p.up ? 1 : 0][s.si];
  ROMA_REQUIRE(seg >= 0 && (size_t)slab * c.nimg == s.pf_bytes, "roma_encode: the pack layout does not hold this scale");
  for (int i0 = 0; i0 < c.nimg && !dry; i0 += SLAB_MAX) {
    SlabTable t;
    t.n = std::min((int)SLAB_MAX, c.nimg - i0);
    for (int k = 0; k < t.n; ++k) t.src_idx[k] = t.dst_idx[k] = i0 + k;
    RUN(slab_copy_launch(s.pf, slab, feats + seg, pack.total, slab, t, c.st));
  }
  return 0;
}

int Model::encode_impl(int n, const float* im, const float* im_hr, char* feats, hipStream_t st, bool dry, bool with_up, Arena& arena,
                       Arena& persist) {
  Call c(arena, persist);
  c.B = n; c.nimg = n; c.shift = 0; c.sym = false; c.ndp = 0;
  c.esz = act_dt == DT_F32 ? 4 : 2;
  c.st = st; c.dry = dry;
  arena.reset();
  persist.reset();
  dbg_cur_slot = 0;
  token_grid(c);
  if (int rc = fits(c)) return rc;
  for (int pass = 0; pass < (with_up ? 2 : 1); ++pass) {
    Pass p;
    p.up = pass == 1;
    p.H = p.up ? cfg.upsample_h : cfg.coarse_h; p.W = p.up ? cfg.upsample_w : cfg.coarse_w;
    p.imA = p.up ? im_hr : im;
    const size_t pass_mark = arena.mark();
    if (int rc = encode_vgg(c, p)) return rc;
    if (!p.up)
      if (int rc = encode_dino(c, p)) return rc;
    for (int si = p.up ? 1 : 0; si < 5; ++si) {
      Scale s(c, p, si, ref[si]);
      const size_t scale_mark = arena.mark();
      if (int rc = proj_head(c, p, s)) return rc;
      if (int rc = scatter_head(c, p, s, feats)) return rc;
      arena.release(scale_mark);
    }
    arena.release(pass_mark);
  }
  return 0;
}

int Model::match_impl(int B, const float* ima, const float* imb, const float* ima_hr, const float* imb_hr,
                      float* warp_out, float* cert_out, hipStream_t st, bool dry, Arena& arena, Arena& persist,
                      const roma_forward_args_t* fw, const EncodedIn* enc) {
  Call c(arena, persist);
  c.B = B; c.nimg = 2 * B; c.shift = B;
  c.sym = fw ? fw->symmetric != 0 : cfg.symmetric != 0;
  c.ndp = c.sym ? 2 * B : B;
  c.esz = act_dt == DT_F32 ? 4 : 2;
  c.st = st; c.dry = dry; c.fw = fw;
  arena.reset();
  persist.reset();
  c.tslot = (&arena == &this->arena) ? 0 : (int)(&arena - side_arena) + 1;
  dbg_cur_slot = c.tslot;
  c.tracing = trace_on && !dry;
  if (c.tracing) {
    if (!trace_dev[c.tslot]) {
      ROMA_CHECK_HIP(hipMalloc((void**)&trace_dev[c.tslot], TRACE_MAX * sizeof(unsigned long long)));
      owned.push_back(trace_dev[c.tslot]);
    }
    ROMA_CHECK_HIP(hipMemsetAsync(trace_dev[c.tslot], 0, TRACE_MAX * sizeof(unsigned long long), st));
    trace_n[c.tslot] = 0;
  }
  token_grid(c);

  float* cert16_keep = (float*)c.alloc((size_t)c.ndp * c.T, 4);
  float *pp_flow[2][2] = {{nullptr, nullptr}, {nullptr, nullptr}}, *pp_cert[2][2] = {{nullptr, nullptr}, {nullptr, nullptr}};
  for (int ps = 0; ps < ((cfg.upsample_preds || (fw && fw->upsample)) ? 2 : 1); ++ps) {
    const size_t px = (size_t)c.ndp * (ps ? cfg.upsample_h : cfg.coarse_h) * (ps ? cfg.upsample_w : cfg.coarse_w);
    for (int i = 0; i < 2; ++i) {
      pp_flow[ps][i] = (float*)c.alloc(px * 2, 4);
      pp_cert[ps][i] = (float*)c.alloc(px, 4);
    }
  }
  if (int rc = fits(c)) return rc;
  float *flow_p1 = nullptr, *cert_p1 = nullptr;
  float *flow_fin = nullptr, *cert_fin = nullptr;

  const int pass0 = fw ? (fw->upsample ? 1 : 0) : 0, pass1 = fw ? pass0 + 1 : (cfg.upsample_preds ? 2 : 1);
  for (int pass = pass0; pass < pass1; ++pass) {
    Pass p;
    p.up = pass == 1;
    p.H = p.up ? cfg.upsample_h : cfg.coarse_h; p.W = p.up ? cfg.upsample_w : cfg.coarse_w;
    p.imA = (p.up && !fw) ? ima_hr : ima;
    p.imB = (p.up && !fw) ? imb_hr : imb;
    p.scale_factor = sqrt((double)p.H * (double)p.W / (560.0 * 560.0));
    if (!p.up && coarse_scale_factor > 0.0) p.scale_factor = coarse_scale_factor;
    if (fw && fw->scale_factor > 0.0) p.scale_factor = fw->scale_factor;
    p.flow = pp_flow[pass][0]; p.cert = pp_cert[pass][0]; p.flow_alt = pp_flow[pass][1]; p.cert_alt = pp_cert[pass][1];

    const size_t pass_mark = arena.mark();
    if (enc) {
      if (!p.up)
        if (int rc = decoder_scratch(c)) return rc;
    } else {
      if (int rc = encode_vgg(c, p)) return rc;
      if (!p.up)
        if (int rc = encode_dino(c, p)) return rc;
    }
    if (p.up)
      if (int rc = seed_upsample_pass(c, p, flow_p1, cert_p1)) return rc;
    for (int si = p.up ? 1 : 0; si < 5; ++si) {
      Scale s(c, p, si, ref[si]);
      const size_t scale_mark = arena.mark();
      if (int rc = enc ? gather_head(c, p, s, *enc) : proj_head(c, p, s)) return rc;
      if (s.ins == 16) {
        const size_t coarse_mark = arena.mark();
        if (int rc = coarse_match(c, p, s)) return rc;
        arena.release(coarse_mark);
      }
      const void* d_last = nullptr;
      bool composed = false;
      if (int rc = refiner_input(c, p, s)) return rc;
      if (int rc = refiner_chain(c, p, s, &d_last, &composed)) return rc;
      if (int rc = refiner_out(c, p, s, d_last, composed)) return rc;
      arena.release(scale_mark);
      if (int rc = next_scale(c, p, s, cert16_keep)) return rc;
    }
    flow_fin = p.flow; cert_fin = p.cert;
    if (!p.up) { flow_p1 = p.flow; cert_p1 = p.cert; }
    arena.release(pass_mark);
  }
  if (fw) return 0;
  return epilogue(c, flow_fin, cert_fin, cert16_keep, warp_out, cert_out);
}

}
```

roma_amd/csrc/tuning.hip:

```cpp
#include "tuning.h"

#include <stdlib.h>
#include <string.h>

#include "../../include/roma_hip.h"

namespace roma {
void set_error(const std::string& msg);
namespace {

struct Row {
  Switch id;
  const char* key;
  const char* env;
  long def;
  int floor;
  const char* doc;
};

constexpr Row ROWS[] = {
    {SW_GEMM8P, "gemm8p", "ROMA_GEMM8P", 1, 0, "large bf16 GEMMs on the 8-phase 256 x 256 kernel (1) or on the one-barrier-per-slab kernel (0)"},
    {SW_GEMM_DBG, "gemm_dbg", "ROMA_GEMM_DBG", 0, 0, "experiment bits of the GEMM kernels (1 skip output stores, 2 skip the K loop, 2048 no streaming stores, ...)"},
    {SW_GEMM8P_WALK, "gemm8p_walk", nullptr, -1, 1, "gemm8p: tile rows per group of the persistent walk (1 = row major); unset = 8 from 24 tile columns on, else 1"},
    {SW_GEMM8P_SCHED, "gemm8p_sched", "ROMA_GEMM8P_SCHED", 1, 0, "gemm8p K-loop schedule: 1 k-half phases, 0 quadrant phases (tools builds only)"},
    {SW_GEMM8P_MAXWG, "gemm8p_maxwg", nullptr, -1, 8, "gemm8p, measurement only: cap the persistent grid at n workgroups (a multiple of 8); unset = one per CU"},
    {SW_WS1X1, "ws1x1", "ROMA_WS1X1", 1, 0, "N = K = 576 refiner 1x1 on the weight-stationary kernel (1) or on the 256 x 192 tile kernel (0)"},
    {SW_LC_MODE, "lc_mode", "ROMA_LC_MODE", 0, 0, "local correlation: 0 tiled form + gather work list, 1 every tile on the gather list (key only), 2 per-pixel kernel"},
    {SW_LC_BIN, "lc_bin", "ROMA_LC_BIN", 1, 0, "local correlation: queries of incoherent tiles sorted by target bin, counters in LDS (1) or device atomics (2), or gathered per query (0)"},
    {SW_CONV64, "conv64", "ROMA_CONV64", 7, 0, "weight-stationary VGG front end, bit mask: 1 the Cin = 64 kernels, 2 the Cin = 128 kernel, 4 the fused first layer"},
    {SW_CONV_PATCH, "conv_patch", "ROMA_CONV_PATCH", 1, 0, "patch-resident 3x3 kernel for slab-major VGG layers (1) or gemm8p (0); environment 0 also packs tap-major weights"},
    {SW_ATTN_XCD, "attn_xcd", "ROMA_ATTN_XCD", 1, 0, "attention work items in per-XCD bands of (batch, head) (1) or in plain order (0)"},
    {SW_ATTN_EXP2, "attn_exp2", nullptr, -1, 0, "tools only: force the 2^x softmax of the 16-bit attention kernel on / off; unset = as the caller says"},
    {SW_DW_RING, "dw_ring", "ROMA_DW_RING", 1, 0, "depthwise 5x5: 0 register-prefetch kernel, 1 ring kernel for the large launches, 2 ring kernel for every shape it takes"},
    {SW_GP_COL, "gp_col", "ROMA_GP_COL", 1, 0, "GP Cholesky left-looking, one launch per block column (1) or the right-looking launch chain (0)"},
    {SW_POOL_PROJ, "pool_proj", "ROMA_POOL_PROJ", 1, 0, "max-pool + proj head of strides 1 / 2 in one pass (1) or as separate kernels (0)"},
    {SW_GP_COL_LEADER, "gp_col_leader", "ROMA_GP_COL_LEADER", 1, 0, "block-column Cholesky: a leader workgroup factorises the diagonal block, its product formed one launch ahead (1) or in its own launch (2), or every workgroup its own copy (0)"},
    {SW_GEMM8P_MINM, nullptr, "ROMA_GEMM8P_MINM", 2048, 0, "gemm8p: smallest M it takes for the wide (N >= 2048) dense launches"},
    {SW_GEMM_NT, nullptr, "ROMA_GEMM_NT", 1, 0, "non-temporal output stores in the 16-bit GEMM row writer"},
    {SW_GEMM_F32_FILL, nullptr, "ROMA_GEMM_F32_FILL", 1, 0, "exact-f32 GEMMs below 192 tiles of 256 x 256 run on 128 x 128 tiles"},
    {SW_GEMM_SMALLM, nullptr, "ROMA_GEMM_SMALLM", 1, 0, "GEMMs below 320 tiles of 128 x 128 run on 128 x 64 tiles"},
    {SW_CONV64_SY, nullptr, "ROMA_CONV64_SY", 0, 0, "conv64 strip height in rows; 0 = the split of H with the fewest rounds"},
    {SW_CONV_KORDER, nullptr, "ROMA_CONV_KORDER", 1, 0, "VGG layers with Cout >= 256 pack slab-major weight rows (read when a handle is created)"},
    {SW_RB_SY, nullptr, "ROMA_RB_SY", 0, 0, "fused refiner block strip height in rows; 0 = the split of H with the fewest rounds"},
    {SW_DWR_MAXSY, nullptr, "ROMA_DWR_MAXSY", 1 << 20, 0, "depthwise ring kernel: cap of the strip height in rows (at least 6)"},
    {SW_DW_RING_MINELEMS, nullptr, "ROMA_DW_RING_MINELEMS", 64l << 20, 0, "dw_ring = 1: smallest launch, in elements, that goes to the ring kernel"},
    {SW_RI_VEC, nullptr, "ROMA_RI_VEC", 1, 0, "refiner_input on the 16-byte vector kernel where alignment allows"},
    {SW_OUT_ROW, nullptr, "ROMA_OUT_ROW", 1, 0, "refiner_out: row kernel for C = 24 in 16-bit storage"},
    {SW_OUT_LPR, nullptr, "ROMA_OUT_LPR", 1, 0, "refiner_out, 16-bit: lanes per row chosen to fill the 16-byte pieces best"},
    {SW_OUT_ROWS_IT, nullptr, "ROMA_OUT_ROWS_IT", 0, 0, "refiner_out: row groups per wave (even, >= 2); otherwise 8"},
    {SW_GP_AUG, nullptr, "ROMA_GP_AUG", 1, 0, "GP Cholesky: right-hand sides stored behind A ride along the factorisation (0 = separate forward loop)"},
    {SW_GP_BWD2, nullptr, "ROMA_GP_BWD2", 1, 0, "GP Cholesky: backward substitution with one launch per step (0 = two)"},
    {SW_COMPOSE_OUT, nullptr, "ROMA_COMPOSE_OUT", 1, 0, "initial value of the handle option compose_out_conv (read when a handle is created)"},
    {SW_VIT_RES_F32, nullptr, "ROMA_VIT_RES_F32", 0, 0, "force DINOv2's f32 residual stream in the 16-bit modes"},
    {SW_STREAMS, nullptr, "ROMA_STREAMS", 0, 0, "number of sub-batch streams of match(); 0 = the handle's option"},
    {SW_STREAMS_SERIAL, nullptr, "ROMA_STREAMS_SERIAL", 0, 0, "diagnostic: sub-batch streams run one after the other"},
    {SW_DEBUG_DUAL_SLOT, nullptr, "ROMA_DEBUG_DUAL_SLOT", -1, 0, "diagnostic: keep the stream split in debug mode, sub-batch k captures the stages of ROMA_DEBUG_ONLY"},
};
constexpr int NROWS = sizeof(ROWS) / sizeof(ROWS[0]);
constexpr bool rows_in_enum_order() {
  for (int i = 0; i < NROWS; ++i)
    if (ROWS[i].id != i) return false;
  return true;
}
static_assert(NROWS == SW_COUNT && rows_in_enum_order(), "one row per Switch, in enum order");
constexpr bool json_plain(const char* s) {
  for (; s && *s; ++s)
    if (*s == '"' || *s == '\\' || *s < ' ') return false;
  return true;
}
constexpr bool rows_json_plain() {
  for (const Row& r : ROWS)
    if (!json_plain(r.key) || !json_plain(r.env) || !json_plain(r.doc)) return false;
  return true;
}
static_assert(rows_json_plain(), "keys, environment names and docs: plain ASCII without quote, backslash or control character");

struct Overrides {
  long v[SW_COUNT];
  constexpr Overrides() : v{} {
    for (long& x : v) x = -1;
  }
};
[[clang::require_constant_initialization]] Overrides g_override;

struct Env {
  long v[SW_COUNT];
  Env() {
    for (int i = 0; i < NROWS; ++i) {
      const char* s = ROWS[i].env ? getenv(ROWS[i].env) : nullptr;
      v[i] = s ? atol(s) : ROWS[i].def;
    }
  }
};
const Env& env() {
  static const Env e;
  return e;
}

}

long tuning_env(Switch id) { return env().v[id]; }
long tuning_override(Switch id) { return g_override.v[id] >= ROWS[id].floor ? g_override.v[id] : -1; }
long tuning(Switch id) { return g_override.v[id] >= ROWS[id].floor ? g_override.v[id] : tuning_env(id); }

int tuning_set(const char* key, long value) {
  for (const Row& r : ROWS)
    if (r.key && !strcmp(r.key, key)) {
      g_override.v[r.id] = value >= r.floor ? value : -1;
      return 0;
    }
  set_error(std::string("roma_tuning: unknown key ") + key);
  return ROMA_ERR_ARG;
}

std::string tuning_describe() {
  std::string js = "[";
  for (const Row& r : ROWS) {
    const auto quoted = [](const char* s) { return s ? "\"" + std::string(s) + "\"" : std::string("null"); };
    const long ov = tuning_override(r.id);
    js += std::string(r.id ? ", " : "") + "{\"key\": " + quoted(r.key) + ", \"env\": " + quoted(r.env) +
          ", \"default\": " + std::to_string(r.def) + ", \"override\": " + (ov >= 0 ? std::to_string(ov) : "null") +
          ", \"value\": " + std::to_string(tuning(r.id)) + ", \"doc\": " + quoted(r.doc) + "}";
  }
  return js + "]";
}

}
```

Baseline: 109.7 image-pairs/s.

## Fuse VGG conv1_1 into the weight-stationary conv1_2 kernel

Adds a fused VGG front-end kernel that computes the 3-channel conv1_1 on the fly, per row strip, inside the weight-stationary Cin=64 conv1_2 kernel. The row-pipelined conv body moves into a shared template header parameterised on a FRONT mode. This removes the intermediate 64-channel full-resolution activation write and read between the two layers, plus one launch. The cost is extra per-block recomputation of conv1_1 on halo columns and rows. It also adds a C entry point that chains the fused front end with pool_proj.

After: 110.2 image-pairs/s, median of 6. No clear change (+0.5%).

```diff
diff --git a/include/roma_hip_vgg_front.h b/include/roma_hip_vgg_front.h
--- /dev/null
+++ b/include/roma_hip_vgg_front.h
@@ -0,0 +1,14 @@
+#ifndef ROMA_HIP_VGG_FRONT_H
+#define ROMA_HIP_VGG_FRONT_H
+#ifdef __cplusplus
+extern "C" {
+#endif
+
+int roma_op_vgg_front(const float* im_a, const float* im_b, const void* w1, const float* b1, const void* w2, const float* b2,
+                      const void* pw, long ldw, const float* pb, int N, int ldf, void* feat, void* pooled, void* pf, int B, int H,
+                      int W, void* stream);
+
+#ifdef __cplusplus
+}
+#endif
+#endif
diff --git a/roma_amd/_lib.py b/roma_amd/_lib.py
--- a/roma_amd/_lib.py
+++ b/roma_amd/_lib.py
@@ -72,6 +72,13 @@
     if _twice:
         raise ImportError(f"{_path} declares {_twice} a second time")
     EXTENSIONS.update(_sigs)
+VGG_FRONT_HEADER = os.path.join(os.path.dirname(_PKG), "include", "roma_hip_vgg_front.h")
+if not os.path.exists(VGG_FRONT_HEADER):
+    raise ImportError(f"{VGG_FRONT_HEADER} not found - roma_amd reads the signatures of the C ABI from it")
+with open(VGG_FRONT_HEADER) as _f:
+    VGG_FRONT = parse_header(_f.read())
+if set(VGG_FRONT) & (set(SIGNATURES) | set(EXTENSIONS)):
+    raise ImportError(f"{VGG_FRONT_HEADER} declares {sorted(set(VGG_FRONT) & (set(SIGNATURES) | set(EXTENSIONS)))} a second time")
 
 _libs = {}
 
@@ -88,7 +95,7 @@
         raise ImportError(f"{path} not found - build it with `python -c 'import __graft_entry__ as g; g.build()'` "
                           "(roma_amd has no CPU fallback)")
     lib = C.CDLL(path)
-    for name, (res, args) in {**SIGNATURES, **EXTENSIONS}.items():
+    for name, (res, args) in {**SIGNATURES, **EXTENSIONS, **VGG_FRONT}.items():
         fn = getattr(lib, name)
         fn.restype = res
         fn.argtypes = args
diff --git a/roma_amd/csrc/conv64.h b/roma_amd/csrc/conv64.h
--- a/roma_amd/csrc/conv64.h
+++ b/roma_amd/csrc/conv64.h
@@ -3,5 +3,9 @@
 
 namespace roma {
 int conv64_try_launch(const GemmArgs& a, hipStream_t stream);
+int conv64_strip_rows(int B, int H, int nxt, int slots);
 int conv3x3_c3_bf16_launch(const float* img, const void* w, const float* bias, void* out, int B, int H, int W, hipStream_t stream);
+bool vgg_front_supported(int H, int W);
+int vgg_front_launch(const float* imA, const float* imB, const void* w1, const float* b1, const void* w2, const float* b2, void* out,
+                     int B, int H, int W, hipStream_t stream);
 }
diff --git a/roma_amd/csrc/conv64.hip b/roma_amd/csrc/conv64.hip
--- a/roma_amd/csrc/conv64.hip
+++ b/roma_amd/csrc/conv64.hip
@@ -5,201 +5,17 @@
 
 #include <algorithm>
 
+#include "conv64_rows.h"
 #include "gemm_device.h"
 #include "tuning.h"
 
 namespace roma {
-
-static __device__ __attribute__((aligned(256))) unsigned int g_c64_dump[256];
-
-#define C64_WAIT_VM(N) asm volatile("s_waitcnt vmcnt(%0)" ::"n"(N) : "memory")
 
 template <int COUT>
 __global__ __launch_bounds__(256, 2) void conv3x3_c64_kernel(const bf16_t* __restrict__ in, const bf16_t* __restrict__ w,
                                                              const float* __restrict__ bias, bf16_t* __restrict__ out, int B,
                                                              int H, int W, int SY, int nxt, int nblocks) {
-  constexpr int NCG = COUT / 32;
-  constexpr int NPG = 4 / NCG;
-  constexpr int TW = 64 * NPG;
-  constexpr int NPIECE = ((TW + 2) * 128 + 1023) / 1024;
-  constexpr int RSTRIDE = NPIECE * 1024;
-  constexpr int KW = (NPIECE + 3) / 4;
-  extern __shared__ __attribute__((aligned(1024))) unsigned char ring[];
-
-  if ((int)blockIdx.x >= nblocks) return;
-  const int tid = threadIdx.x, lane = tid & 63;
-  const int wave = __builtin_amdgcn_readfirstlane(tid >> 6);
-  const int cg = wave % NCG, pg = wave / NCG;
-  const int l31 = lane & 31, h = lane >> 5;
-  typedef unsigned u32x4 __attribute__((ext_vector_type(4)));
-  const unsigned ring0 = (unsigned)(size_t)((__attribute__((address_space(3))) unsigned char*)ring);
-
-  u32x4 wreg[36];
-  {
-    const bf16_t* wp = w + (long)(32 * cg + l31) * 576 + 8 * h;
-#pragma unroll
-    for (int ks = 0; ks < 36; ++ks) wreg[ks] = *reinterpret_cast<const u32x4*>(wp + 16 * ks);
-  }
-  float* bias_s = reinterpret_cast<float*>(ring + 4 * RSTRIDE);
-  if (tid < COUT) bias_s[tid] = bias[tid];
-
-  unsigned rdo[3];
-#pragma unroll
-  for (int dx = 0; dx < 3; ++dx) {
-    const int p = 64 * pg + l31 + dx;
-    rdo[dx] = ring0 + (unsigned)(p * 128 + ((h ^ ((p >> 1) & 7)) << 4));
-  }
-
-  for (int lb = blockIdx.x; lb < nblocks; lb += gridDim.x) {
-  const int xt = lb % nxt;
-  const int r = lb / nxt;
-  const int yt = (H + SY - 1) / SY;
-  const int ys = (r % yt) * SY;
-  const int b = r / yt;
-  const int x0 = xt * TW;
-  const int sy = min(SY, H - ys);
-  if (lb != (int)blockIdx.x) __builtin_amdgcn_s_barrier();
-
-  const bf16_t* inb = in + (long)b * H * W * 64;
-  const __amdgpu_buffer_rsrc_t rs_in = __builtin_amdgcn_make_buffer_rsrc(const_cast<bf16_t*>(inb), 0, (int)((long)H * W * 128), 0x00020000);
-  unsigned voff[KW];
-  bool okx[KW];
-  {
-    const int dl_p = lane >> 3, dl_slot = lane & 7;
-    const u32x4 z4 = {0u, 0u, 0u, 0u};
-#pragma unroll
-    for (int j = 0; j < KW; ++j) {
-      const int q = wave + 4 * j;
-      const int p = q * 8 + dl_p;
-      const int x = x0 - 1 + p;
-      const int c = dl_slot ^ ((p >> 1) & 7);
-      okx[j] = q < NPIECE && p < TW + 2 && x >= 0 && x < W;
-      voff[j] = okx[j] ? (unsigned)(x * 128 + c * 16) : 0u;
-      if (q < NPIECE && !okx[j]) {
-        int ln = lane;
-        asm volatile("" : "+v"(ln));
-#pragma unroll
-        for (int sl = 0; sl < 4; ++sl)
-          asm volatile("ds_write_b128 %0, %1" ::"v"(ring0 + sl * RSTRIDE + q * 1024 + ln * 16), "v"(z4) : "memory");
-      }
-    }
-  }
-  asm volatile("s_waitcnt vmcnt(0) lgkmcnt(0)" ::: "memory");
-
-#define C64_ISSUE_ROW(YY, SLOT)                                                                                \
-  {                                                                                                            \
-    const int yy_ = (YY);                                                                                      \
-    if (yy_ >= 0 && yy_ < H) {                                                                                 \
-      const int so_ = yy_ * W * 128;                                                                           \
-      _Pragma("unroll") for (int j = 0; j < KW; ++j) {                                                         \
-        const int q_ = wave + 4 * j;                                                                           \
-        if (q_ < NPIECE) {                                                                                     \
-          if (okx[j])                                                                                          \
-            __builtin_amdgcn_raw_ptr_buffer_load_lds(rs_in, (__attribute__((address_space(3))) void*)(ring + (SLOT) * RSTRIDE + q_ * 1024), \
-                                                     16, (int)voff[j], so_, 0, 0);                             \
-        }                                                                                                      \
-      }                                                                                                        \
-    } else {                                     \
-      const u32x4 z4_ = {0u, 0u, 0u, 0u};                                                                      \
-      int ln_ = lane;                                                                                          \
-      asm volatile("" : "+v"(ln_));                                                                            \
-      _Pragma("unroll") for (int j = 0; j < KW; ++j) {                                                         \
-        const int q_ = wave + 4 * j;                                                                           \
-        if (q_ < NPIECE)                                                                                       \
-          asm volatile("ds_write_b128 %0, %1" ::"v"(ring0 + (SLOT) * RSTRIDE + q_ * 1024 + ln_ * 16), "v"(z4_) : "memory"); \
-      }                                                                                                        \
-    }                                                                                                          \
-  }
-
-  u32x4 fa[2][4];
-#define C64_READ_G(SLOTOFF, DX, G)                                                                            \
-  {                                                                                                           \
-    const unsigned ad_ = (rdo[DX] + (SLOTOFF)) ^ (unsigned)((G) << 5);                                         \
-    asm volatile("ds_read_b128 %0, %1" : "=v"(fa[0][G]) : "v"(ad_));                                           \
-    asm volatile("ds_read_b128 %0, %1 offset:4096" : "=v"(fa[1][G]) : "v"(ad_));                              \
-  }
-#define C64_WAIT_G(G, N) asm volatile("s_waitcnt lgkmcnt(%2)" : "+v"(fa[0][G]), "+v"(fa[1][G]) : "n"(N) : "memory")
-
-  C64_ISSUE_ROW(ys - 1, 0)
-  C64_ISSUE_ROW(ys, 1)
-  C64_ISSUE_ROW(ys + 1, 2)
-
-  bf16_t* outb = out + (long)b * H * W * COUT;
-  for (int o = 0; o < sy; ++o) {
-    if (o == 0) {
-      asm volatile("s_waitcnt vmcnt(0) lgkmcnt(0)" ::: "memory");
-    } else {
-      C64_WAIT_VM(0);
-    }
-    __builtin_amdgcn_s_barrier();
-    C64_ISSUE_ROW(ys + o + 2, (o + 3) & 3)
-    if (o == 0) {
-      C64_READ_G(0, 0, 0)
-      C64_READ_G(0, 0, 1)
-    }
-    C64_READ_G((o & 3) * RSTRIDE, 0, 2)
-    C64_READ_G((o & 3) * RSTRIDE, 0, 3)
-
-    f32x16 acc[2];
-#pragma unroll
-    for (int tm = 0; tm < 2; ++tm)
-#pragma unroll
-      for (int e = 0; e < 16; ++e) acc[tm][e] = 0.f;
-#pragma unroll
-    for (int t = 0; t < 9; ++t) {
-#pragma unroll
-      for (int g = 0; g < 4; ++g) {
-        if (t == 8 && g == 3) {
-          C64_WAIT_G(g, 4);
-        } else {
-          C64_WAIT_G(g, 6);
-        }
-#pragma unroll
-        for (int tm = 0; tm < 2; ++tm)
-          acc[tm] = mfma_h16_32x32x16(wreg[t * 4 + g],
-                                                            fa[tm][g], acc[tm]);
-        __builtin_amdgcn_sched_barrier(0);
-        if (t + 1 < 9) {
-          C64_READ_G(((o + (t + 1) / 3) & 3) * RSTRIDE, (t + 1) % 3, g)
-        } else if (g < 2) {
-          C64_READ_G(((o + 1) & 3) * RSTRIDE, 0, g)
-        }
-        __builtin_amdgcn_sched_barrier(0);
-      }
-    }
-
-    const int y = ys + o;
-#pragma unroll
-    for (int P = 0; P < 2; ++P) {
-      f32x4 bv0, bv1;
-      {
-        const unsigned ba = ring0 + 4 * RSTRIDE + (32 * cg + 16 * P + 4 * h) * 4;
-        asm volatile("ds_read_b128 %0, %2\n\tds_read_b128 %1, %2 offset:32\n\ts_waitcnt lgkmcnt(0)"
-                     : "=&v"(bv0), "=&v"(bv1)
-                     : "v"(ba)
-                     : "memory");
-      }
-#pragma unroll
-      for (int tm = 0; tm < 2; ++tm) {
-        const int x = x0 + 64 * pg + 32 * tm + l31;
-        const unsigned a0 = pack_bf16x2(fmaxf(acc[tm][8 * P + 0] + bv0[0], 0.f), fmaxf(acc[tm][8 * P + 1] + bv0[1], 0.f));
-        const unsigned a1 = pack_bf16x2(fmaxf(acc[tm][8 * P + 2] + bv0[2], 0.f), fmaxf(acc[tm][8 * P + 3] + bv0[3], 0.f));
-        const unsigned b0 = pack_bf16x2(fmaxf(acc[tm][8 * P + 4] + bv1[0], 0.f), fmaxf(acc[tm][8 * P + 5] + bv1[1], 0.f));
-        const unsigned b1 = pack_bf16x2(fmaxf(acc[tm][8 * P + 6] + bv1[2], 0.f), fmaxf(acc[tm][8 * P + 7] + bv1[3], 0.f));
-        const auto s0 = __builtin_amdgcn_permlane32_swap(a0, b0, false, false);
-        const auto s1 = __builtin_amdgcn_permlane32_swap(a1, b1, false, false);
-        const u32x4 st = {s0[0], s1[0], s0[1], s1[1]};
-        bf16_t* op = outb + ((long)y * W + x) * COUT + 32 * cg + 16 * P + 8 * h;
-        u32x4* dst = x < W ? reinterpret_cast<u32x4*>(op) : reinterpret_cast<u32x4*>(g_c64_dump) + lane;
-        *dst = st;
-      }
-    }
-  }
-  C64_WAIT_VM(0);
-  }
-#undef C64_WAIT_G
-#undef C64_READ_G
-#undef C64_ISSUE_ROW
+  conv64_rows<COUT, false>(in, C64Front{}, w, bias, out, B, H, W, SY, nxt, nblocks);
 }
 
 template <int DUMMY>
@@ -474,36 +290,15 @@
       }
     }
     u32x4 fr[2];
-#pragma unroll
-    for (int ks = 0; ks < 2; ++ks)
-#pragma unroll
-      for (int j = 0; j < 4; ++j) fr[ks][j] = pack_bf16x2(v[8 * ks + 2 * j], v[8 * ks + 2 * j + 1]);
-    f32x16 acc[2];
+    conv1_1_taps(v, fr);
 #pragma unroll
     for (int cb = 0; cb < 2; ++cb) {
-#pragma unroll
-      for (int e = 0; e < 16; ++e) acc[cb][e] = 0.f;
-#pragma unroll
-      for (int ks = 0; ks < 2; ++ks)
-        acc[cb] = mfma_h16_32x32x16(wf[cb][ks],
-                                                          fr[ks], acc[cb]);
-    }
-#pragma unroll
-    for (int cb = 0; cb < 2; ++cb)
-#pragma unroll
-      for (int P = 0; P < 2; ++P) {
-        const f32x4 b0 = *reinterpret_cast<const f32x4*>(bias_s + 32 * cb + 16 * P + 4 * h);
-        const f32x4 b1 = *reinterpret_cast<const f32x4*>(bias_s + 32 * cb + 16 * P + 8 + 4 * h);
-        const unsigned a0 = pack_bf16x2(fmaxf(acc[cb][8 * P + 0] + b0[0], 0.f), fmaxf(acc[cb][8 * P + 1] + b0[1], 0.f));
-        const unsigned a1 = pack_bf16x2(fmaxf(acc[cb][8 * P + 2] + b0[2], 0.f), fmaxf(acc[cb][8 * P + 3] + b0[3], 0.f));
-        const unsigned c0 = pack_bf16x2(fmaxf(acc[cb][8 * P + 4] + b1[0], 0.f), fmaxf(acc[cb][8 * P + 5] + b1[1], 0.f));
-        const unsigned c1 = pack_bf16x2(fmaxf(acc[cb][8 * P + 6] + b1[2], 0.f), fmaxf(acc[cb][8 * P + 7] + b1[3], 0.f));
-        const auto s0 = __builtin_amdgcn_permlane32_swap(a0, c0, false, false);
-        const auto s1 = __builtin_amdgcn_permlane32_swap(a1, c1, false, false);
-        const u32x4 st = {s0[0], s1[0], s0[1], s1[1]};
-        const int c = 4 * cb + 2 * P + h;
-        *reinterpret_cast<__attribute__((address_space(3))) u32x4*>(st0 + l31 * 128 + ((c ^ (l31 & 7)) << 4)) = st;
-      }
+      u32x4 st2[2];
+      conv1_1_block(fr, wf[cb], bias_s, cb, h, st2);
+#pragma unroll
+      for (int P = 0; P < 2; ++P)
+        *reinterpret_cast<__attribute__((address_space(3))) u32x4*>(st0 + l31 * 128 + (((4 * cb + 2 * P + h) ^ (l31 & 7)) << 4)) = st2[P];
+    }
 #pragma unroll
     for (int i = 0; i < 4; ++i) {
       const u32x4 st = *reinterpret_cast<__attribute__((address_space(3))) const u32x4*>(st0 + i * 1024 + lane * 16);
@@ -525,6 +320,23 @@
                      reinterpret_cast<const bf16_t*>(w), bias, reinterpret_cast<bf16_t*>(out), B, H, W, RY, nxt, ntiles);
   ROMA_LAUNCH_CHECK();
   return 0;
+}
+
+int conv64_strip_rows(int B, int H, int nxt, int slots) {
+  int SY = (int)tuning(SW_CONV64_SY);
+  if (SY <= 0) {
+    long best = -1;
+    for (int yt = 1; yt <= std::max(1, H / 12); ++yt) {
+      const int sy = (H + yt - 1) / yt;
+      const long n = (long)B * nxt * ((H + sy - 1) / sy);
+      const long cost = ((n + slots - 1) / slots) * (sy + 3);
+      if (best < 0 || cost < best) {
+        best = cost;
+        SY = sy;
+      }
+    }
+  }
+  return SY;
 }
 
 int conv64_try_launch(const GemmArgs& a, hipStream_t stream) {
@@ -542,21 +354,8 @@
   const int B = (int)(a.M / hw);
   const int TW = (!c128 && a.N == 64) ? 128 : 64;
   const int slots = c128 ? 256 : 512;
-  const int sy_env = tuning(SW_CONV64_SY);
   const int nxt = (W + TW - 1) / TW;
-  int SY = sy_env;
-  if (SY <= 0) {
-    long best = -1;
-    for (int yt = 1; yt <= std::max(1, H / 12); ++yt) {
-      const int sy = (H + yt - 1) / yt;
-      const long n = (long)B * nxt * ((H + sy - 1) / sy);
-      const long cost = ((n + slots - 1) / slots) * (sy + 3);
-      if (best < 0 || cost < best) {
-        best = cost;
-        SY = sy;
-      }
-    }
-  }
+  const int SY = conv64_strip_rows(B, H, nxt, slots);
   const long nb = (long)B * ((H + SY - 1) / SY) * nxt;
   if (nb <= 0 || nb >= (1l << 30)) return 1;
   char pname[64];
diff --git a/roma_amd/csrc/conv64_rows.h b/roma_amd/csrc/conv64_rows.h
--- /dev/null
+++ b/roma_amd/csrc/conv64_rows.h
@@ -0,0 +1,362 @@
+#pragma once
+#include "gemm_device.h"
+
+namespace roma {
+
+static __device__ __attribute__((aligned(256))) unsigned int g_c64_dump[256];
+
+#define C64_WAIT_VM(N) asm volatile("s_waitcnt vmcnt(%0)" ::"n"(N) : "memory")
+
+typedef unsigned c64_u32x4 __attribute__((ext_vector_type(4)));
+
+__device__ __forceinline__ void conv1_1_taps(const float (&v)[16], c64_u32x4 (&fr)[2]) {
+#pragma unroll
+  for (int ks = 0; ks < 2; ++ks)
+#pragma unroll
+    for (int j = 0; j < 4; ++j) fr[ks][j] = pack_bf16x2(v[8 * ks + 2 * j], v[8 * ks + 2 * j + 1]);
+}
+__device__ __forceinline__ void conv1_1_block(const c64_u32x4 (&fr)[2], const c64_u32x4 (&wf)[2], const float* bias_s, int cb, int h,
+                                              c64_u32x4 (&st)[2]) {
+  f32x16 acc;
+#pragma unroll
+  for (int e = 0; e < 16; ++e) acc[e] = 0.f;
+#pragma unroll
+  for (int ks = 0; ks < 2; ++ks) acc = mfma_h16_32x32x16(wf[ks], fr[ks], acc);
+#pragma unroll
+  for (int P = 0; P < 2; ++P) {
+    const f32x4 b0 = *reinterpret_cast<const f32x4*>(bias_s + 32 * cb + 16 * P + 4 * h);
+    const f32x4 b1 = *reinterpret_cast<const f32x4*>(bias_s + 32 * cb + 16 * P + 8 + 4 * h);
+    const unsigned a0 = pack_bf16x2(fmaxf(acc[8 * P + 0] + b0[0], 0.f), fmaxf(acc[8 * P + 1] + b0[1], 0.f));
+    const unsigned a1 = pack_bf16x2(fmaxf(acc[8 * P + 2] + b0[2], 0.f), fmaxf(acc[8 * P + 3] + b0[3], 0.f));
+    const unsigned c0 = pack_bf16x2(fmaxf(acc[8 * P + 4] + b1[0], 0.f), fmaxf(acc[8 * P + 5] + b1[1], 0.f));
+    const unsigned c1 = pack_bf16x2(fmaxf(acc[8 * P + 6] + b1[2], 0.f), fmaxf(acc[8 * P + 7] + b1[3], 0.f));
+    const auto s0 = __builtin_amdgcn_permlane32_swap(a0, c0, false, false);
+    const auto s1 = __builtin_amdgcn_permlane32_swap(a1, c1, false, false);
+    st[P] = c64_u32x4{s0[0], s1[0], s0[1], s1[1]};
+  }
+}
+
+struct C64Front {
+  const float* imA;
+  const float* imB;
+  const bf16_t* w1;
+  const float* b1;
+  int B;
+};
+
+constexpr int C64F_TW = 126, C64F_RING = 4 * 17 * 1024;
+constexpr int C64F_IMW = C64F_TW + 4, C64F_IMN = 3 * C64F_IMW, C64F_IMP = (C64F_IMN + 63) / 64, C64F_IMS = C64F_IMP * 256;
+constexpr int C64F_IMR = C64F_RING + 512, C64F_W1 = C64F_IMR + 4 * C64F_IMS, C64F_LDS = C64F_W1 + 64 * 32 * 2;
+
+template <int COUT, bool FRONT>
+__device__ __forceinline__ void conv64_rows(const bf16_t* __restrict__ in, const C64Front fr, const bf16_t* __restrict__ w,
+                                            const float* __restrict__ bias, bf16_t* __restrict__ out, int B, int H, int W, int SY,
+                                            int nxt, int nblocks) {
+  static_assert(!FRONT || COUT == 64, "the FRONT form is conv1_1 -> conv1_2");
+  constexpr int NCG = COUT / 32;
+  constexpr int NPG = 4 / NCG;
+  constexpr int TW = 64 * NPG;
+  constexpr int TWO = FRONT ? C64F_TW : TW;
+  constexpr int NPIECE = ((TW + 2) * 128 + 1023) / 1024;
+  constexpr int RSTRIDE = NPIECE * 1024;
+  constexpr int KW = (NPIECE + 3) / 4;
+  extern __shared__ __attribute__((aligned(1024))) unsigned char ring[];
+
+  if ((int)blockIdx.x >= nblocks) return;
+  const int tid = threadIdx.x, lane = tid & 63;
+  const int wave = __builtin_amdgcn_readfirstlane(tid >> 6);
+  const int cg = wave % NCG, pg = wave / NCG;
+  const int l31 = lane & 31, h = lane >> 5;
+  typedef c64_u32x4 u32x4;
+  const unsigned ring0 = (unsigned)(size_t)((__attribute__((address_space(3))) unsigned char*)ring);
+
+  u32x4 wreg[36];
+  {
+    const bf16_t* wp = w + (long)(32 * cg + l31) * 576 + 8 * h;
+#pragma unroll
+    for (int ks = 0; ks < 36; ++ks) wreg[ks] = *reinterpret_cast<const u32x4*>(wp + 16 * ks);
+  }
+  float* bias_s = reinterpret_cast<float*>(ring + 4 * RSTRIDE);
+  if (tid < COUT) bias_s[tid] = bias[tid];
+  if constexpr (FRONT) {
+    static_assert(4 * RSTRIDE == C64F_RING, "LDS map of the FRONT form");
+    if (tid < 64) bias_s[64 + tid] = fr.b1[tid];
+    reinterpret_cast<u32x4*>(ring + C64F_W1)[tid] = reinterpret_cast<const u32x4*>(fr.w1)[tid];
+  }
+
+  unsigned rdo[3];
+#pragma unroll
+  for (int dx = 0; dx < 3; ++dx) {
+    const int p = 64 * pg + l31 + dx;
+    rdo[dx] = ring0 + (unsigned)(p * 128 + ((h ^ ((p >> 1) & 7)) << 4));
+  }
+
+  for (int lb = blockIdx.x; lb < nblocks; lb += gridDim.x) {
+  const int xt = lb % nxt;
+  const int r = lb / nxt;
+  const int yt = (H + SY - 1) / SY;
+  const int ys = (r % yt) * SY;
+  const int b = r / yt;
+  const int x0 = xt * TWO;
+  const int sy = min(SY, H - ys);
+  if (lb != (int)blockIdx.x) __builtin_amdgcn_s_barrier();
+
+  const bf16_t* inb = FRONT ? nullptr : in + (long)b * H * W * 64;
+  const __amdgpu_buffer_rsrc_t rs_in = __builtin_amdgcn_make_buffer_rsrc(const_cast<bf16_t*>(inb), 0, FRONT ? 0 : (int)((long)H * W * 128), 0x00020000);
+  unsigned voff[KW];
+  bool okx[KW];
+  {
+    const int dl_p = lane >> 3, dl_slot = lane & 7;
+    const u32x4 z4 = {0u, 0u, 0u, 0u};
+#pragma unroll
+    for (int j = 0; j < KW; ++j) {
+      const int q = wave + 4 * j;
+      const int p = q * 8 + dl_p;
+      const int x = x0 - 1 + p;
+      const int c = dl_slot ^ ((p >> 1) & 7);
+      okx[j] = q < NPIECE && p < TWO + 2 && x >= 0 && x < W;
+      voff[j] = okx[j] ? (unsigned)(x * 128 + c * 16) : 0u;
+      if (q < NPIECE && !okx[j]) {
+        int ln = lane;
+        asm volatile("" : "+v"(ln));
+#pragma unroll
+        for (int sl = 0; sl < 4; ++sl)
+          asm volatile("ds_write_b128 %0, %1" ::"v"(ring0 + sl * RSTRIDE + q * 1024 + ln * 16), "v"(z4) : "memory");
+      }
+    }
+  }
+  constexpr int KI = FRONT ? (C64F_IMP + 3) / 4 : 1;
+  const long HW = (long)H * W;
+  const float* imb = nullptr;
+  if constexpr (FRONT) imb = b < fr.B ? fr.imA + (long)b * 3 * HW : fr.imB + (long)(b - fr.B) * 3 * HW;
+  const __amdgpu_buffer_rsrc_t rs_img = __builtin_amdgcn_make_buffer_rsrc(const_cast<float*>(imb), 0, FRONT ? (int)(HW * 12) : 0, 0x00020000);
+  const unsigned imr0 = ring0 + C64F_IMR;
+  unsigned ivoff[KI];
+  bool oki[KI];
+  if constexpr (FRONT) {
+#pragma unroll
+    for (int j = 0; j < KI; ++j) {
+      const int q = wave + 4 * j;
+      const int e = q * 64 + lane;
+      const int ch = e / C64F_IMW, x = x0 - 2 + e % C64F_IMW;
+      oki[j] = q < C64F_IMP && e < C64F_IMN && x >= 0 && x < W;
+      ivoff[j] = oki[j] ? (unsigned)(((long)ch * HW + x) * 4) : 0u;
+      if (q < C64F_IMP && !oki[j]) {
+        int ln = lane;
+        asm volatile("" : "+v"(ln));
+#pragma unroll
+        for (int sl = 0; sl < 4; ++sl)
+          asm volatile("ds_write_b32 %0, %1" ::"v"(imr0 + sl * C64F_IMS + q * 256 + ln * 4), "v"(0u) : "memory");
+      }
+    }
+  }
+  asm volatile("s_waitcnt vmcnt(0) lgkmcnt(0)" ::: "memory");
+
+#define C64_ZERO_ROW(SLOT)                                                                                     \
+  {                                                                                                            \
+    const u32x4 z4_ = {0u, 0u, 0u, 0u};                                                                        \
+    int ln_ = lane;                                                                                            \
+    asm volatile("" : "+v"(ln_));                                                                              \
+    _Pragma("unroll") for (int j = 0; j < KW; ++j) {                                                           \
+      const int q_ = wave + 4 * j;                                                                             \
+      if (q_ < NPIECE)                                                                                         \
+        asm volatile("ds_write_b128 %0, %1" ::"v"(ring0 + (SLOT) * RSTRIDE + q_ * 1024 + ln_ * 16), "v"(z4_) : "memory"); \
+    }                                                                                                          \
+  }
+#define C64_ISSUE_ROW(YY, SLOT)                                                                                \
+  {                                                                                                            \
+    const int yy_ = (YY);                                                                                      \
+    if (yy_ >= 0 && yy_ < H) {                                                                                 \
+      const int so_ = yy_ * W * 128;                                                                           \
+      _Pragma("unroll") for (int j = 0; j < KW; ++j) {                                                         \
+        const int q_ = wave + 4 * j;                                                                           \
+        if (q_ < NPIECE) {                                                                                     \
+          if (okx[j])                                                                                          \
+            __builtin_amdgcn_raw_ptr_buffer_load_lds(rs_in, (__attribute__((address_space(3))) void*)(ring + (SLOT) * RSTRIDE + q_ * 1024), \
+                                                     16, (int)voff[j], so_, 0, 0);                             \
+        }                                                                                                      \
+      }                                                                                                        \
+    } else C64_ZERO_ROW(SLOT)                                                                                  \
+  }
+#define C64_ISSUE_IMG(YY)                                                                                      \
+  {                                                                                                            \
+    const int yy_ = (YY);                                                                                      \
+    const int sl_ = (yy_ - ys) & 3;                                                                            \
+    if (yy_ >= 0 && yy_ < H) {                                                                                 \
+      const int so_ = yy_ * W * 4;                                                                             \
+      _Pragma("unroll") for (int j = 0; j < KI; ++j) {                                                         \
+        const int q_ = wave + 4 * j;                                                                           \
+        if (q_ < C64F_IMP) {                                                                                   \
+          if (oki[j])                                                                                          \
+            __builtin_amdgcn_raw_ptr_buffer_load_lds(rs_img, (__attribute__((address_space(3))) void*)(ring + C64F_IMR + sl_ * C64F_IMS + q_ * 256), \
+                                                     4, (int)ivoff[j], so_, 0, 0);                             \
+        }                                                                                                      \
+      }                                                                                                        \
+    } else {                                                                                                   \
+      int ln_ = lane;                                                                                          \
+      asm volatile("" : "+v"(ln_));                                                                            \
+      _Pragma("unroll") for (int j = 0; j < KI; ++j) {                                                         \
+        const int q_ = wave + 4 * j;                                                                           \
+        if (q_ < C64F_IMP)                                                                                     \
+          asm volatile("ds_write_b32 %0, %1" ::"v"(imr0 + sl_ * C64F_IMS + q_ * 256 + ln_ * 4), "v"(0u) : "memory"); \
+      }                                                                                                        \
+    }                                                                                                          \
+  }
+#define C64_PRODUCE_ROW(YY, SLOT)                                                                              \
+  {                                                                                                            \
+    const int yy_ = (YY);                                                                                      \
+    if (yy_ >= 0 && yy_ < H) {                                                                                 \
+      unsigned srow_[3];                                                                                       \
+      _Pragma("unroll") for (int ky = 0; ky < 3; ++ky) srow_[ky] = imr0 + ((yy_ + ky - 1 - ys) & 3) * C64F_IMS; \
+      {                                                                                                        \
+        int ln_ = lane;  \
+        asm volatile("" : "+v"(ln_));                                                                          \
+        const int l31_ = ln_ & 31, h_ = ln_ >> 5;                                                              \
+        const int p_ = 32 * wave + l31_;                                                                       \
+        const int pr_ = p_ * 4;                                                                                \
+        const int x_ = x0 - 1 + p_;                                                                            \
+        float v_[16];                                                                                          \
+        _Pragma("unroll") for (int s_ = 0; s_ < 16; ++s_) {                                                    \
+          const int k0_ = s_, k1_ = 16 + s_ < 27 ? 16 + s_ : 0;                             \
+          const unsigned a0_ = srow_[(k0_ % 9) / 3] + ((k0_ / 9) * C64F_IMW + k0_ % 3) * 4;                    \
+          const unsigned a1_ = srow_[(k1_ % 9) / 3] + ((k1_ / 9) * C64F_IMW + k1_ % 3) * 4;                    \
+          const float ld_ = *(__attribute__((address_space(3))) const float*)(size_t)((h_ ? a1_ : a0_) + pr_);   \
+          v_[s_] = (h_ && 16 + s_ >= 27) ? 0.f : ld_;         \
+        }                                                                                                      \
+        u32x4 fr_[2];                                                                                          \
+        conv1_1_taps(v_, fr_);                                                                                 \
+        const bool ok_ = x_ >= 0 && x_ < W;                                                                    \
+        _Pragma("unroll") for (int cb = 0; cb < 2; ++cb) {                                                     \
+          u32x4 wf_[2], st_[2];                                                                                \
+          _Pragma("unroll") for (int ks = 0; ks < 2; ++ks)                                                     \
+            wf_[ks] = *(__attribute__((address_space(3))) const u32x4*)(size_t)(ring0 + C64F_W1 + 32 * cb * 64 + (l31_ * 64 + 32 * h_) + 16 * ks); \
+          conv1_1_block(fr_, wf_, bias_s + 64, cb, h_, st_);                                                   \
+          if (ok_) {                                                                                           \
+            _Pragma("unroll") for (int P = 0; P < 2; ++P)                                                      \
+              asm volatile("ds_write_b128 %0, %1" ::"v"(ring0 + (SLOT) * RSTRIDE + p_ * 128 + (((4 * cb + 2 * P + h_) ^ ((p_ >> 1) & 7)) << 4)), \
+                           "v"(st_[P]) : "memory");                                                            \
+          }                                                                                                    \
+          __builtin_amdgcn_sched_barrier(0);  \
+        }                                                                                                      \
+      }                                                                                                        \
+    } else C64_ZERO_ROW(SLOT)                                                                                  \
+  }
+
+  u32x4 fa[2][4];
+#define C64_READ_G(SLOTOFF, DX, G)                                                                            \
+  {                                                                                                           \
+    const unsigned ad_ = (rdo[DX] + (SLOTOFF)) ^ (unsigned)((G) << 5);                                         \
+    asm volatile("ds_read_b128 %0, %1" : "=v"(fa[0][G]) : "v"(ad_));                                           \
+    asm volatile("ds_read_b128 %0, %1 offset:4096" : "=v"(fa[1][G]) : "v"(ad_));                              \
+  }
+#define C64_WAIT_G(G, N) asm volatile("s_waitcnt lgkmcnt(%2)" : "+v"(fa[0][G]), "+v"(fa[1][G]) : "n"(N) : "memory")
+
+  if constexpr (FRONT) {
+    C64_ISSUE_IMG(ys - 2)
+    C64_ISSUE_IMG(ys - 1)
+    C64_ISSUE_IMG(ys)
+    C64_ISSUE_IMG(ys + 1)
+    asm volatile("s_waitcnt vmcnt(0) lgkmcnt(0)" ::: "memory");
+    __builtin_amdgcn_s_barrier();
+    C64_PRODUCE_ROW(ys - 1, 0)
+    C64_PRODUCE_ROW(ys, 1)
+    asm volatile("s_waitcnt lgkmcnt(0)" ::: "memory");
+    __builtin_amdgcn_s_barrier();
+    C64_ISSUE_IMG(ys + 2)
+    C64_ISSUE_IMG(ys + 3)
+    asm volatile("s_waitcnt vmcnt(0) lgkmcnt(0)" ::: "memory");
+    __builtin_amdgcn_s_barrier();
+    C64_PRODUCE_ROW(ys + 1, 2)
+  } else {
+    C64_ISSUE_ROW(ys - 1, 0)
+    C64_ISSUE_ROW(ys, 1)
+    C64_ISSUE_ROW(ys + 1, 2)
+  }
+
+  bf16_t* outb = out + (long)b * H * W * COUT;
+  for (int o = 0; o < sy; ++o) {
+    if (FRONT || o == 0) {
+      asm volatile("s_waitcnt vmcnt(0) lgkmcnt(0)" ::: "memory");
+    } else {
+      C64_WAIT_VM(0);
+    }
+    __builtin_amdgcn_s_barrier();
+    if constexpr (FRONT) {
+      if (o + 2 <= sy) C64_PRODUCE_ROW(ys + o + 2, (o + 3) & 3)
+      if (o + 3 <= sy) C64_ISSUE_IMG(ys + o + 4)
+    } else {
+      C64_ISSUE_ROW(ys + o + 2, (o + 3) & 3)
+    }
+    if (o == 0) {
+      C64_READ_G(0, 0, 0)
+      C64_READ_G(0, 0, 1)
+    }
+    C64_READ_G((o & 3) * RSTRIDE, 0, 2)
+    C64_READ_G((o & 3) * RSTRIDE, 0, 3)
+
+    f32x16 acc[2];
+#pragma unroll
+    for (int tm = 0; tm < 2; ++tm)
+#pragma unroll
+      for (int e = 0; e < 16; ++e) acc[tm][e] = 0.f;
+#pragma unroll
+    for (int t = 0; t < 9; ++t) {
+#pragma unroll
+      for (int g = 0; g < 4; ++g) {
+        if (t == 8 && g == 3) {
+          C64_WAIT_G(g, 4);
+        } else {
+          C64_WAIT_G(g, 6);
+        }
+#pragma unroll
+        for (int tm = 0; tm < 2; ++tm)
+          acc[tm] = mfma_h16_32x32x16(wreg[t * 4 + g],
+                                                            fa[tm][g], acc[tm]);
+        __builtin_amdgcn_sched_barrier(0);
+        if (t + 1 < 9) {
+          C64_READ_G(((o + (t + 1) / 3) & 3) * RSTRIDE, (t + 1) % 3, g)
+        } else if (g < 2) {
+          C64_READ_G(((o + 1) & 3) * RSTRIDE, 0, g)
+        }
+        __builtin_amdgcn_sched_barrier(0);
+      }
+    }
+
+    const int y = ys + o;
+#pragma unroll
+    for (int P = 0; P < 2; ++P) {
+      f32x4 bv0, bv1;
+      {
+        const unsigned ba = ring0 + 4 * RSTRIDE + (32 * cg + 16 * P + 4 * h) * 4;
+        asm volatile("ds_read_b128 %0, %2\n\tds_read_b128 %1, %2 offset:32\n\ts_waitcnt lgkmcnt(0)"
+                     : "=&v"(bv0), "=&v"(bv1)
+                     : "v"(ba)
+                     : "memory");
+      }
+#pragma unroll
+      for (int tm = 0; tm < 2; ++tm) {
+        const int x = x0 + 64 * pg + 32 * tm + l31;
+        const unsigned a0 = pack_bf16x2(fmaxf(acc[tm][8 * P + 0] + bv0[0], 0.f), fmaxf(acc[tm][8 * P + 1] + bv0[1], 0.f));
+        const unsigned a1 = pack_bf16x2(fmaxf(acc[tm][8 * P + 2] + bv0[2], 0.f), fmaxf(acc[tm][8 * P + 3] + bv0[3], 0.f));
+        const unsigned b0 = pack_bf16x2(fmaxf(acc[tm][8 * P + 4] + bv1[0], 0.f), fmaxf(acc[tm][8 * P + 5] + bv1[1], 0.f));
+        const unsigned b1 = pack_bf16x2(fmaxf(acc[tm][8 * P + 6] + bv1[2], 0.f), fmaxf(acc[tm][8 * P + 7] + bv1[3], 0.f));
+        const auto s0 = __builtin_amdgcn_permlane32_swap(a0, b0, false, false);
+        const auto s1 = __builtin_amdgcn_permlane32_swap(a1, b1, false, false);
+        const u32x4 st = {s0[0], s1[0], s0[1], s1[1]};
+        bf16_t* op = outb + ((long)y * W + x) * COUT + 32 * cg + 16 * P + 8 * h;
+        u32x4* dst = x < W && (!FRONT || 64 * pg + 32 * tm + l31 < TWO) ? reinterpret_cast<u32x4*>(op) : reinterpret_cast<u32x4*>(g_c64_dump) + lane;
+        *dst = st;
+      }
+    }
+  }
+  C64_WAIT_VM(0);
+  }
+#undef C64_WAIT_G
+#undef C64_READ_G
+#undef C64_PRODUCE_ROW
+#undef C64_ISSUE_IMG
+#undef C64_ISSUE_ROW
+#undef C64_ZERO_ROW
+}
+
+}
diff --git a/roma_amd/csrc/model.hip b/roma_amd/csrc/model.hip
--- a/roma_amd/csrc/model.hip
+++ b/roma_amd/csrc/model.hip
@@ -380,7 +380,12 @@
   void* t1 = c.alloc((size_t)nimg * (H / 2) * (W / 2) * 64, esz);
   void* col1 = c.alloc((size_t)nimg * H * W * 32, esz);
   if (int rc = fits(c)) return rc;
-  if (act_dt == DT_BF16 && (tuning(SW_CONV64) & 4) && (long)3 * H * W < (1l << 23)) {
+  const long c64 = tuning(SW_CONV64);
+  const bool front = act_dt == DT_BF16 && (c64 & 1) && (c64 & 4) && !(c64 & 8) && !c.fw && !debug && !c.tracing &&
+                     vgg[1].ldw == 576 && vgg_korder[1] == 0 && vgg_front_supported(H, W);
+  if (front) {
+    RUN(vgg_front_launch(p.imA, p.imB, vgg[0].w, vgg[0].b, vgg[1].w, vgg[1].b, p.feat[0], B, H, W, st));
+  } else if (act_dt == DT_BF16 && (c64 & 4) && (long)3 * H * W < (1l << 23)) {
     RUN(conv3x3_c3_bf16_launch(p.imA, vgg[0].w, vgg[0].b, t0, B, H, W, st));
     if (p.imB) RUN(conv3x3_c3_bf16_launch(p.imB, vgg[0].w, vgg[0].b, c.at(t0, (long)B * H * W * 64), B, H, W, st));
   } else {
@@ -410,7 +415,8 @@
     }
     return 0;
   };
-  if (int rc = conv(1, t0, p.feat[0], H, W)) return rc;
+  if (!front)
+    if (int rc = conv(1, t0, p.feat[0], H, W)) return rc;
   if (int rc = pool(0, p.feat[0], t1)) return rc;
   if (int rc = conv(2, t1, t0, H / 2, W / 2)) return rc;
   if (int rc = conv(3, t0, p.feat[1], H / 2, W / 2)) return rc;
diff --git a/roma_amd/csrc/tuning.hip b/roma_amd/csrc/tuning.hip
--- a/roma_amd/csrc/tuning.hip
+++ b/roma_amd/csrc/tuning.hip
@@ -27,7 +27,7 @@
     {SW_WS1X1, "ws1x1", "ROMA_WS1X1", 1, 0, "N = K = 576 refiner 1x1 on the weight-stationary kernel (1) or on the 256 x 192 tile kernel (0)"},
     {SW_LC_MODE, "lc_mode", "ROMA_LC_MODE", 0, 0, "local correlation: 0 tiled form + gather work list, 1 every tile on the gather list (key only), 2 per-pixel kernel"},
     {SW_LC_BIN, "lc_bin", "ROMA_LC_BIN", 1, 0, "local correlation: queries of incoherent tiles sorted by target bin, counters in LDS (1) or device atomics (2), or gathered per query (0)"},
-    {SW_CONV64, "conv64", "ROMA_CONV64", 7, 0, "weight-stationary VGG front end, bit mask: 1 the Cin = 64 kernels, 2 the Cin = 128 kernel, 4 the fused first layer"},
+    {SW_CONV64, "conv64", "ROMA_CONV64", 7, 0, "weight-stationary VGG front end, bit mask: 1 the Cin = 64 kernels, 2 the Cin = 128 kernel, 4 the fused first layer, 8 conv1_1 as a kernel of its own in match() (0 = inside conv1_2)"},
     {SW_CONV_PATCH, "conv_patch", "ROMA_CONV_PATCH", 1, 0, "patch-resident 3x3 kernel for slab-major VGG layers (1) or gemm8p (0); environment 0 also packs tap-major weights"},
     {SW_ATTN_XCD, "attn_xcd", "ROMA_ATTN_XCD", 1, 0, "attention work items in per-XCD bands of (batch, head) (1) or in plain order (0)"},
     {SW_ATTN_EXP2, "attn_exp2", nullptr, -1, 0, "tools only: force the 2^x softmax of the 16-bit attention kernel on / off; unset = as the caller says"},
diff --git a/roma_amd/csrc/vgg_front.hip b/roma_amd/csrc/vgg_front.hip
--- /dev/null
+++ b/roma_amd/csrc/vgg_front.hip
@@ -0,0 +1,55 @@
+#include <algorithm>
+
+#include "../../include/roma_hip_vgg_front.h"
+#include "conv64.h"
+#include "conv64_rows.h"
+#include "pool_proj.h"
+
+namespace roma {
+
+__global__ __launch_bounds__(256, 2) void vgg_front_kernel(const float* __restrict__ imA, const float* __restrict__ imB, int Bh,
+                                                           const bf16_t* __restrict__ w1, const float* __restrict__ b1,
+                                                           const bf16_t* __restrict__ w2, const float* __restrict__ b2,
+                                                           bf16_t* __restrict__ out, int nimg, int H, int W, int SY, int nxt,
+                                                           int nblocks) {
+  conv64_rows<64, true>(nullptr, C64Front{imA, imB, w1, b1, Bh}, w2, b2, out, nimg, H, W, SY, nxt, nblocks);
+}
+
+bool vgg_front_supported(int H, int W) { return H > 0 && W > 0 && (long)H * W * 128 < (1l << 31); }
+
+int vgg_front_launch(const float* imA, const float* imB, const void* w1, const float* b1, const void* w2, const float* b2, void* out,
+                     int B, int H, int W, hipStream_t stream) {
+  ROMA_REQUIRE(imA && w1 && b1 && w2 && b2 && out && B > 0, "vgg_front: bad arguments");
+  ROMA_REQUIRE(vgg_front_supported(H, W), "vgg_front: H * W * 128 bytes must stay below 2^31");
+  const int nimg = imB ? 2 * B : B;
+  const int slots = 512;
+  const int nxt = (W + C64F_TW - 1) / C64F_TW;
+  const int SY = conv64_strip_rows(nimg, H, nxt, slots);
+  const long nb = (long)nimg * ((H + SY - 1) / SY) * nxt;
+  ROMA_REQUIRE(nb > 0 && nb < (1l << 30), "vgg_front: grid too large");
+  ProfScope ps("vgg_front_kernel", 2.0 * (double)nimg * H * W * 64 * (576.0 + 27.0), "flop", stream);
+  static bool attr_set[64] = {false};
+  int dev = 0;
+  ROMA_CHECK_HIP(hipGetDevice(&dev));
+  if (dev < 0 || dev >= 64 || !attr_set[dev]) {
+    ROMA_CHECK_HIP(hipFuncSetAttribute(reinterpret_cast<const void*>(&vgg_front_kernel), hipFuncAttributeMaxDynamicSharedMemorySize, C64F_LDS));
+    if (dev >= 0 && dev < 64) attr_set[dev] = true;
+  }
+  hipLaunchKernelGGL(vgg_front_kernel, dim3((unsigned)std::min<long>(nb, slots)), dim3(256), C64F_LDS, stream, imA, imB, B,
+                     reinterpret_cast<const bf16_t*>(w1), b1, reinterpret_cast<const bf16_t*>(w2), b2, reinterpret_cast<bf16_t*>(out),
+                     nimg, H, W, SY, nxt, (int)nb);
+  ROMA_LAUNCH_CHECK();
+  return 0;
+}
+
+}
+
+using namespace roma;
+
+extern "C" int roma_op_vgg_front(const float* im_a, const float* im_b, const void* w1, const float* b1, const void* w2,
+                                 const float* b2, const void* pw, long ldw, const float* pb, int N, int ldf, void* feat,
+                                 void* pooled, void* pf, int B, int H, int W, void* stream) {
+  ROMA_REQUIRE(feat && pooled && pf && pw && pb, "roma_op_vgg_front: null pointer");
+  if (int rc = vgg_front_launch(im_a, im_b, w1, b1, w2, b2, feat, B, H, W, (hipStream_t)stream)) return rc;
+  return pool_proj_launch(feat, pooled, pf, pw, ldw, pb, N, ldf, im_b ? 2 * B : B, H, W, 64, DT_BF16, (hipStream_t)stream);
+}
```
